# MMintLab/gelslim_depth

Hardware: AMD Instinct MI355X
Metric: train frames/sec (320x427) at batch 32 (higher is better)
Workload: dtype f32

## Files before the change

### gelslim_depth_amd/_lib.py

```python
from __future__ import annotations

import ctypes as C
import os
from typing import Optional, Sequence, Tuple

import torch

_HERE = os.path.dirname(os.path.abspath(__file__))
LIB_PATH = os.environ.get("GSD_LIB_PATH") or os.path.join(_HERE, "csrc", "libgsd.so")


class GsdError(RuntimeError):
    pass


class gsd_src(C.Structure):
    _fields_ = [("ptr", C.c_void_p), ("scale", C.c_void_p), ("shift", C.c_void_p),
                ("C", C.c_int32), ("H", C.c_int32), ("W", C.c_int32),
                ("off_h", C.c_int32), ("off_w", C.c_int32), ("relu", C.c_int32),
                ("w_stride", C.c_int32), ("slack", C.c_int32),
                ("n_stride", C.c_int64), ("c_stride", C.c_int64)]


class gsd_dst(C.Structure):
    _fields_ = [("ptr", C.c_void_p), ("C", C.c_int32), ("H", C.c_int32), ("W", C.c_int32),
                ("off_h", C.c_int32), ("off_w", C.c_int32), ("w_stride", C.c_int32),
                ("n_stride", C.c_int64), ("c_stride", C.c_int64)]


class gsd_guard(C.Structure):
    _fields_ = [("words", C.c_void_p), ("tick", C.c_int32)]


class gsd_nhwc(C.Structure):
    _fields_ = [("ptr", C.c_void_p), ("pitch", C.c_int64),
                ("N", C.c_int32), ("H", C.c_int32), ("W", C.c_int32), ("C", C.c_int32)]


_P = C.c_void_p
_I = C.c_int
_L = C.c_int64
_F = C.c_float
_D = C.c_double
_SRC = C.POINTER(gsd_src)
_DST = C.POINTER(gsd_dst)
_GUARD = C.POINTER(gsd_guard)
class gsd_bf16_bnbwd(C.Structure):
    _fields_ = [("y", C.POINTER(gsd_nhwc)), ("scale", C.c_void_p), ("shift", C.c_void_p), ("mean", C.c_void_p),
                ("invstd", C.c_void_p)]


class gsd_wl_job(C.Structure):
    _fields_ = [("w", C.c_void_p), ("wt", C.c_void_p), ("mode", C.c_int32), ("Co", C.c_int32), ("Ci", C.c_int32), ("reserved", C.c_int32)]


class gsd_bf16_wimg_job(C.Structure):
    _fields_ = [("w", C.c_void_p), ("out", C.c_void_p), ("mode", C.c_int32), ("Cout", C.c_int32), ("Cin", C.c_int32),
                ("reserved", C.c_int32)]


_NHWC = C.POINTER(gsd_nhwc)
_BNBWD = C.POINTER(gsd_bf16_bnbwd)
_IP = C.POINTER(C.c_int)

SIGNATURES = {
    "gsd_version": (C.c_char_p, []),
    "gsd_last_error": (C.c_char_p, []),
    "gsd_selftest_mfma": (_I, [_P, _P, _P, _P]),
    "gsd_weight_layout_size": (_L, [_I, _I, _I]),
    "gsd_weight_layout": (_I, [_I, _P, _I, _I, _P, _P]),
    "gsd_weight_layout_batch": (_I, [C.POINTER(gsd_wl_job), _I, _P]),
    "gsd_conv3x3_partial_rows": (_I, [_I, _I, _I, _I]),
    "gsd_conv3x3": (_I, [_SRC, _I, _P, _I, _I, _DST, _I, _P, _I, _I, _I, _P]),
    "gsd_conv3x3_dgrad_bnrelu": (_I, [_SRC, _P, _I, _I, _DST, _P, _P, _P, _P, _P, _P, _I, _I, _I, _P]),
    "gsd_conv3x3_algo": (_I, [_I, _I, _I, _I, _I]),
    "gsd_conv3x3_w43_partial_rows": (_I, [_I, _I, _I, _I]),
    "gsd_conv3x3_w43_mfma_count": (C.c_int64, [_I, _I, _I, _I, _I]),
    "gsd_conv3x3_w43": (_I, [_SRC, _I, _P, _I, _I, _DST, _I, _P, _I, _I, _I, _P]),
    "gsd_conv3x3_w43_dgrad_bnrelu": (_I, [_SRC, _P, _I, _I, _DST, _P, _P, _P, _P, _P, _P, _I, _I, _I, _P]),
    "gsd_conv3x3_w2d_supported": (_I, [_I, _I]),
    "gsd_conv3x3_prefers_w2d": (_I, [_I, _I, _I, _I, _I, _I]),
    "gsd_conv3x3_w2d_estimate_us": (C.c_double, [_I, _I, _I, _I, _I]),
    "gsd_conv3x3_w43_estimate_us": (C.c_double, [_I, _I, _I, _I, _I, _I]),
    "gsd_conv3x3_w2d_partial_rows": (_I, [_I, _I, _I, _I]),
    "gsd_conv3x3_w2d_mfma_count": (C.c_int64, [_I, _I, _I, _I, _I]),
    "gsd_conv3x3_w2d": (_I, [_SRC, _I, _P, _I, _I, _DST, _I, _P, _I, _I, _I, _P]),
    "gsd_conv3x3_w2d_dgrad_bnrelu": (_I, [_SRC, _P, _I, _I, _DST, _P, _P, _P, _P, _P, _P, _I, _I, _I, _P]),
    "gsd_conv3x3_w2d_estimate_slabs_us": (C.c_double, [_I, _I, _I, _I, _I]),
    "gsd_conv3x3_w2d_workspace": (_L, [_I, _I, _I, _I, _I]),
    "gsd_conv3x3_w2d_ws": (_I, [_SRC, _I, _P, _I, _I, _DST, _I, _P, _P, _L, _I, _I, _I, _P]),
    "gsd_conv3x3_w2d_dgrad_bnrelu_ws": (_I, [_SRC, _P, _I, _I, _DST, _P, _P, _P, _P, _P, _P, _P, _L, _I, _I, _I, _P]),
    "gsd_conv3x3_w43_workspace": (_L, [_I, _I, _I, _I, _I]),
    "gsd_conv3x3_w43_ws": (_I, [_SRC, _I, _P, _I, _I, _DST, _I, _P, _P, _L, _I, _I, _I, _P]),
    "gsd_conv3x3_w43_dgrad_bnrelu_ws": (_I, [_SRC, _P, _I, _I, _DST, _P, _P, _P, _P, _P, _P, _P, _L, _I, _I, _I, _P]),
    "gsd_convT2x2": (_I, [_SRC, _P, _P, _I, _I, _DST, _I, _I, _I, _P]),
    "gsd_convT2x2_dgrad_layout": (_I, [_SRC, _I, _I, _I, _I, _I]),
    "gsd_convT2x2_dgrad": (_I, [_SRC, _P, _I, _I, _DST, _I, _I, _I, _P]),
    "gsd_convT2x2_dgrad_as": (_I, [_I, _SRC, _P, _I, _I, _DST, _I, _I, _I, _P]),
    "gsd_convT2x2_dgrad_bnrelu_partial_rows": (_I, [_SRC, _I, _I, _I, _I, _I]),
    "gsd_convT2x2_dgrad_bnrelu": (_I, [_SRC, _P, _I, _I, _DST, _P, _P, _P, _P, _P, _P, _I, _I, _I, _P]),
    "gsd_conv3x3_wgrad_workspace": (_L, [_I, _I, _I, _I, _I]),
    "gsd_conv3x3_wgrad": (_I, [_SRC, _I, _SRC, _I, _I, _P, _P, _L, _I, _I, _I, _P]),
    "gsd_conv3x3_wgrad_form": (_I, [_SRC, _I, _SRC, _I, _I, _I, _I, _I]),
    "gsd_conv3x3_wgrad_mfma_count": (C.c_int64, [_I, _I, _I, _I, _I, _I]),
    "gsd_conv3x3_wgrad_takes_pitched_dy": (_I, [_I, _I, _I, _I, _I]),
    "gsd_conv3x3_wgrad_bn_supported": (_I, [_I, _I, _I, _I, _I]),
    "gsd_conv3x3_wgrad_bn_workspace": (_L, [_I, _I, _I, _I, _I]),
    "gsd_conv3x3_wgrad_bn": (_I, [_SRC, _P, _P, _P, _P, _P, _P, _P, _I, _I, _P, _P, _L, _I, _I, _I, _P]),
    "gsd_conv3x3_dgrad_bn_supported": (_I, [_I, _I, _I, _I, _I]),
    "gsd_conv3x3_dgrad_bn": (_I, [_P, _P, _P, _P, _P, _P, _P, _P, _I, _I, _P, _I, _I, _I, _P]),
    "gsd_convT2x2_wgrad_workspace": (_L, [_I, _I, _I, _I, _I]),
    "gsd_convT2x2_wgrad": (_I, [_SRC, _SRC, _I, _I, _P, _P, _P, _L, _I, _I, _I, _P]),
    "gsd_bn_reduce_partials": (_I, [_P, _I, _I, _I, _P, _P]),
    "gsd_partials_channel_sums": (_I, [_P, _I, _I, _I, _I, _I, _P, _P, _P]),
    "gsd_add_counters": (_I, [C.POINTER(C.c_void_p), _I, _L, _P]),
    "gsd_bn_finalize": (_I, [_P, _I, _D, _P, _P, _F, _F, _P, _P, _P, _P, _P, _P, _GUARD, _P]),
    "gsd_bn_eval_coeffs": (_I, [_P, _P, _P, _P, _F, _I, _P, _P, _P]),
    "gsd_bn_eval_coeffs_bwd": (_I, [_P, _P, _P, _P, _F, _I, _P, _P, _P, _P, _P]),
    "gsd_bn_bwd_partial_rows": (_I, [_I, _I, _I, _I]),
    "gsd_bn_bwd_reduce": (_I, [_I, _P, _P, _P, _P, _P, _SRC, _P, _P, _P, _I, _P, _P, _I, _I, _I, _I, _P]),
    "gsd_bn_bwd_reduce_partials": (_I, [_P, _I, _I, _P, _P]),
    "gsd_bn_bwd_finalize": (_I, [_P, _P, _I, _D, _P, _P, _P, _P, _P, _P]),
    "gsd_bn_bwd_apply": (_I, [_P, _P, _P, _P, _P, _P, _P, _I, _I, _I, _I, _P, _I, _P]),
    "gsd_sum_planes": (_I, [_P, _I, _I, _L, _P, _P, _P]),
    "gsd_maxpool2": (_I, [_SRC, _P, _I, _I, _I, _I, _P]),
    "gsd_conv1x1_out": (_I, [_SRC, _P, _P, _I, _I, _P, _I, _I, _I, _P]),
    "gsd_conv1x1_out_wgrad_rows": (_I, [_I, _I, _I]),
    "gsd_conv1x1_out_wgrad": (_I, [_P, _P, _P, _P, _I, _I, _P, _P, _P, _I, _I, _I, _P]),
    "gsd_loss_fwd_bwd": (_I, [_I, _P, _P, _L, _F, _P, _P, _P, _GUARD, _P]),
    "gsd_guard_snapshot": (_I, [_P, _P, _L, _P]),
    "gsd_guard_restore": (_I, [_GUARD, _P, _P, _L, _P]),
    "gsd_adam_ema": (_I, [_P, _P, _P, _P, _P, _L, _I, _F, _F, _F, _F, _F, _F, _F, _GUARD, _P]),
    "gsd_bn_reduce_finalize": (_I, [_P, _I, _I, _I, _P, _D, _P, _P, _F, _F, _P, _P, _P, _P, _P, _P, _GUARD, _P]),
    "gsd_bn_bwd_reduce_finalize": (_I, [_P, _I, _I, _I, _P, _D, _P, _P, _P, _P, _P, _P]),
    "gsd_area_resize_affine": (_I, [_P, _P, _I, _I, _I, _I, _P, _I, _I, _P, _P, _I, _F, _F, _P]),
    "gsd_ingest_images": (_I, [_P, _P, _I, _I, _I, _I, _I, _L, _L, _L, _L, _P, _I, _I, _F, _F, _P]),
    "gsd_resize_affine": (_I, [_I, _P, _P, _I, _I, _I, _I, _P, _I, _I, _P, _P, _I, _F, _F, _P]),
    "gsd_ingest_images_interp": (_I, [_I, _P, _P, _I, _I, _I, _I, _I, _L, _L, _L, _L, _P, _I, _I, _F, _F, _P]),
    "gsd_gaussian_blur": (_I, [_P, _L, _I, _I, _P, _I, _P, _P]),
    "gsd_channel_stats_workspace": (_L, [_I]),
    "gsd_channel_stats": (_I, [_P, _L, _I, _L, _P, _P, _P]),
    "gsd_gather_affine": (_I, [_P, _P, _L, _I, _I, _L, _P, _P, _I, _P, _P]),
    "gsd_bf16_conv_mpad": (_I, [_I]),
    "gsd_bf16_conv_partial_rows": (_I, [_I, _I, _I, _I]),
    "gsd_bf16_conv_dense_partial_rows": (_I, [_I, _I, _I, _I, _I, _I, _I]),
    "gsd_bf16_conv3x3": (_I, [_NHWC, _P, _NHWC, _I, _I, _P, _BNBWD, _P]),
    "gsd_bf16_conv_dense": (_I, [_NHWC, _P, _NHWC, _I, _I, _I, _I, _IP, _IP, _I, _I, _I, _I, _I, _P, _P, _BNBWD, _P]),
    "gsd_bf16_conv3x3_bnrelu": (_I, [_NHWC, _P, _NHWC, _I, _I, _P, _P, _P]),
    "gsd_bf16_conv1x1_bnrelu": (_I, [_NHWC, _P, _NHWC, _I, _I, _P, _P, _P]),
    "gsd_bf16_weight_image_size": (_L, [_I, _I, _I]),
    "gsd_bf16_weight_image": (_I, [_I, _P, _I, _I, _P, _P]),
    "gsd_bf16_weight_images": (_I, [C.POINTER(gsd_bf16_wimg_job), _I, _P]),
    "gsd_bf16_im2col3x3": (_I, [_P, _I, _I, _I, _I, _NHWC, _P]),
    "gsd_bf16_conv3x3_first_supported": (_I, [_I, _I]),
    "gsd_bf16_conv3x3_first_partial_rows": (_I, [_I, _I, _I, _I]),
    "gsd_bf16_conv3x3_first": (_I, [_P, _I, _I, _I, _I, _P, _NHWC, _I, _P, _P, _P, _P]),
    "gsd_bf16_wgrad_first_workspace": (_L, [_I, _I, _I, _I]),
    "gsd_bf16_wgrad_first": (_I, [_P, _I, _I, _I, _I, _NHWC, _NHWC, _P, _P, _P, _P, _P, _P, _P, _L, _P]),
    "gsd_bf16_inc_supported": (_I, [_I, _I]),
    "gsd_bf16_inc_conv_partial_rows": (_I, [_I, _I, _I]),
    "gsd_bf16_inc_conv": (_I, [_P, _I, _I, _I, _I, _P, _P, _P, _P, _NHWC, _NHWC, _P, _P]),
    "gsd_bf16_first_bn_bwd_reduce": (_I, [_P, _I, _I, _I, _I, _P, _NHWC, _P, _P, _P, _P, _P, _P]),
    "gsd_bf16_wgrad_first_recompute": (_I, [_P, _I, _I, _I, _I, _P, _NHWC, _P, _P, _P, _P, _P, _P, _P, _P, _L, _P]),
    "gsd_bf16_conv3x3_c64_supported": (_I, [_I, _I]),
    "gsd_bf16_conv3x3_c64_partial_rows": (_I, [_I, _I, _I]),
    "gsd_bf16_conv3x3_c64": (_I, [_NHWC, _P, _NHWC, _P, _BNBWD, _P]),
    "gsd_bf16_bn_apply": (_I, [_NHWC, _P, _P, _NHWC, _I, _P]),
    "gsd_bf16_bn_apply_pool": (_I, [_NHWC, _P, _P, _NHWC, _NHWC, _P]),
    "gsd_bf16_bn_apply_pool_idx": (_I, [_NHWC, _P, _P, _NHWC, _NHWC, _P, _P]),
    "gsd_bf16_bn_bwd_reduce_pool_idx": (_I, [_NHWC, _P, _P, _P, _P, _NHWC, _P, _NHWC, _NHWC, _P, _P]),
    "gsd_bf16_maxpool2": (_I, [_NHWC, _NHWC, _P]),
    "gsd_bf16_conv1x1_out": (_I, [_NHWC, _P, _P, _I, _P, _P]),
    "gsd_bf16_bn_relu_conv1x1_out": (_I, [_NHWC, _P, _P, _P, _P, _I, _P, _P]),
    "gsd_bf16_bn_bwd_partial_rows": (_I, [_I, _I, _I]),
    "gsd_bf16_bn_bwd_reduce": (_I, [_I, _NHWC, _P, _P, _P, _P, _NHWC, _NHWC, _NHWC, _P, _P, _NHWC, _P, _P]),
    "gsd_bf16_bn_bwd_apply": (_I, [_NHWC, _NHWC, _P, _P, _P, _P, _P, _P]),
    "gsd_bf16_channel_sums_workspace": (_L, [_I, _I, _I, _I]),
    "gsd_bf16_channel_sums": (_I, [_NHWC, _I, _I, _I, _I, _P, _P, _L, _P]),
    "gsd_bf16_convT_bias_grad_workspace": (_L, [_I, _I, _I, _I, _I, _I, _I, _I]),
    "gsd_bf16_convT_bias_grad": (_I, [_P, _I, _I, _I, _NHWC, _I, _I, _I, _I, _P, _P, _L, _P]),
    "gsd_bf16_wgrad_workspace": (_L, [_I, _I, _I, _I, _I, _I]),
    "gsd_bf16_wgrad": (_I, [_NHWC, _NHWC, _I, _I, _IP, _IP, _P, _I, _P, _L, _P]),
}


def _load() -> C.CDLL:
    if not os.path.exists(LIB_PATH):
        raise GsdError(
            f"{LIB_PATH} not found: build it first (python -c 'import __graft_entry__ as g; g.build()' "
            f"or python -m gelslim_depth_amd.build). There is no CPU/torch fallback for the hot path.")
    lib = C.CDLL(LIB_PATH)
    for name, (res, args) in SIGNATURES.items():
        fn = getattr(lib, name)
        fn.restype = res
        fn.argtypes = args
    return lib


lib = _load()


def check(rc: int, what: str = "") -> None:
    if rc != 0:
        msg = lib.gsd_last_error().decode("utf-8", "replace")
        raise GsdError(f"libgsd {what} failed (code {rc}): {msg}")


def version() -> str:
    return lib.gsd_version().decode()


def stream_ptr() -> int:
    return torch.cuda.current_stream().cuda_stream


def ptr(t: Optional[torch.Tensor]) -> Optional[int]:
    return None if t is None else t.data_ptr()


def _chk_f32(t: torch.Tensor) -> None:
    if t.dtype != torch.float32 or not t.is_cuda:
        raise GsdError(f"expected a float32 CUDA(HIP) tensor, got {t.dtype} on {t.device}")


def _nchw_strides(t: torch.Tensor) -> Tuple[int, int, int]:
    if t.dim() != 4:
        raise GsdError(f"expected an NCHW tensor, got shape {tuple(t.shape)}")
    n, c, h, w = t.shape
    if w > 1 and t.stride(3) != 1:
        raise GsdError(f"expected an NCHW tensor with unit column stride, got shape {tuple(t.shape)} strides {t.stride()}")
    ws = t.stride(2) if (h > 1 or t.stride(2) >= w) else w
    cs = t.stride(1) if (c > 1 or t.stride(1) >= h * ws) else h * ws
    ns = t.stride(0) if (n > 1 or t.stride(0) >= c * cs) else c * cs
    if ws < w or cs < h * ws or ns < c * cs:
        raise GsdError(f"expected an NCHW tensor with unit column stride, got shape {tuple(t.shape)} strides {t.stride()}")
    return ns, cs, ws


def _chk_nchw(t: torch.Tensor) -> None:
    _nchw_strides(t)


def pitched_empty(shape, device, pitch_multiple: int = 4) -> torch.Tensor:
    n, c, h, w = shape
    p = -(-w // pitch_multiple) * pitch_multiple
    return torch.empty((n, c, h, p), device=device, dtype=torch.float32)[..., :w]


def make_src(t: torch.Tensor, scale: Optional[torch.Tensor] = None, shift: Optional[torch.Tensor] = None,
             relu: bool = False, c_off: int = 0, c_len: Optional[int] = None,
             off: Tuple[int, int] = (0, 0), slack: int = 0) -> gsd_src:
    _chk_f32(t)
    ns, cs, ws = _nchw_strides(t)
    n, ct, h, w = t.shape
    cl = ct - c_off if c_len is None else c_len
    s = gsd_src()
    s.ptr = t.data_ptr() + 4 * c_off * cs
    s.scale = ptr(scale)
    s.shift = ptr(shift)
    s.C, s.H, s.W = cl, h, w
    s.off_h, s.off_w = off
    s.relu = 1 if relu else 0
    s.w_stride = ws
    s.slack = slack
    s.n_stride = ns
    s.c_stride = cs
    return s


SLACK = 4


def slack_empty(shape, device) -> torch.Tensor:
    numel = 1
    for d in shape:
        numel *= int(d)
    buf = torch.empty((numel + 2 * SLACK,), device=device, dtype=torch.float32)
    buf[:SLACK].zero_()
    buf[-SLACK:].zero_()
    return buf[SLACK:SLACK + numel].view(*shape)


def make_dst(t: torch.Tensor, c_off: int = 0, c_len: Optional[int] = None, off: Tuple[int, int] = (0, 0)) -> gsd_dst:
    _chk_f32(t)
    ns, cs, ws = _nchw_strides(t)
    n, ct, h, w = t.shape
    cl = ct - c_off if c_len is None else c_len
    d = gsd_dst()
    d.ptr = t.data_ptr() + 4 * c_off * cs
    d.C, d.H, d.W = cl, h, w
    d.off_h, d.off_w = off
    d.w_stride = ws
    d.n_stride = ns
    d.c_stride = cs
    return d


def make_nhwc(t: torch.Tensor, c_off: int = 0, c_len: Optional[int] = None) -> gsd_nhwc:
    if t.dtype != torch.bfloat16 or not t.is_cuda or t.dim() != 4 or not t.is_contiguous():
        raise GsdError(f"expected a contiguous (N,H,W,C) bfloat16 CUDA(HIP) tensor, got {t.dtype} {tuple(t.shape)} on {t.device}")
    n, h, w, ct = t.shape
    d = gsd_nhwc()
    d.ptr = t.data_ptr() + 2 * c_off
    d.pitch = ct
    d.N, d.H, d.W = n, h, w
    d.C = ct - c_off if c_len is None else c_len
    return d


def make_guard(words: Optional[torch.Tensor], tick: int):
    if words is None:
        return None
    if words.dtype != torch.int32 or not words.is_cuda or words.numel() < 2 or tick == 0:
        raise GsdError("a guard needs two int32 words on the GPU and a non-zero tick")
    g = gsd_guard()
    g.words = words.data_ptr()
    g.tick = tick
    return C.pointer(g)


def add_counters(tensors: Sequence[torch.Tensor], delta: int = 1) -> None:
    if not tensors:
        return
    for t in tensors:
        if t.dtype != torch.int64 or not t.is_cuda or t.numel() != 1:
            raise GsdError(f"add_counters: expected int64 scalars on the GPU, got {t.dtype} {tuple(t.shape)} on {t.device}")
    arr = (C.c_void_p * len(tensors))(*[t.data_ptr() for t in tensors])
    check(lib.gsd_add_counters(arr, len(tensors), delta, stream_ptr()), "add_counters")


def int_array(vals: Sequence[int]):
    return (C.c_int * len(vals))(*vals)


def src_array(items: Sequence[gsd_src]):
    arr = (gsd_src * len(items))()
    for i, it in enumerate(items):
        arr[i] = it
    return arr


def dst_array(items: Sequence[gsd_dst]):
    arr = (gsd_dst * len(items))()
    for i, it in enumerate(items):
        arr[i] = it
    return arr
```

### gelslim_depth_amd/csrc/gsd_conv3x3_w2d.hip

```cpp
#include "gsd_common.h"

#include <cstdio>
#include <cstdlib>
#include <type_traits>

__device__ const float gsd_pad_w2d[2] = {0.f, __builtin_nanf("")};

typedef float f32x4v __attribute__((ext_vector_type(4), aligned(4)));
typedef float f32x2v __attribute__((ext_vector_type(2)));

struct W2DParams {
  SrcD src0, src1;
  DstD dst0, dst1;
  const float* wt;
  float* partials;
  const float* bw_raw;
  const float* bw_scale;
  const float* bw_shift;
  const float* bw_mean;
  const float* bw_invstd;
  int Cin, Cout, Mpad, nchunks, mblocks;
  int N, H, W;
  int TH, TW, TWq, tiles_y, tiles_x, WR, WC, WCp, PS, NPV;
  int NP, NI;
  int mgrp, pgrp, ptiles;
  int nslab;
  float* slabs;
};

namespace {
constexpr int W2D_BM = 64;
constexpr int W2D_WTILE = 96 * W2D_BM;
constexpr int NWP = 2;
}

template <class GetY>
__device__ __forceinline__ void w2d_epilogue(const W2DParams& P, const float* sBw, const int n, const int h0, const int w0, const int tr2,
                                             const int tq, const int vmask, const int m0, const int mh, const int ph, const int j,
                                             const int l16, const int pt, GetY get_y) {
  constexpr int BM = 64;
  int off0_0 = 0, off0_1 = 0, off1_0 = 0, off1_1 = 0, sm0_0 = 0, sm0_1 = 0, sm1_0 = 0, sm1_1 = 0;
#pragma unroll
  for (int a = 0; a < 2; ++a) {
    const int h = h0 + 2 * tr2 + a, w = w0 + 4 * tq;
    const int vm = (vmask >> (4 * a)) & 15;
    int hd = h - P.dst0.oh, wd = w - P.dst0.ow;
    if ((unsigned)hd < (unsigned)P.dst0.H) {
      (a == 0 ? off0_0 : off0_1) = hd * P.dst0.ws + wd;
#pragma unroll
      for (int i = 0; i < 4; ++i)
        if ((vm >> i & 1) && (unsigned)(wd + i) < (unsigned)P.dst0.W) (a == 0 ? sm0_0 : sm0_1) |= 1 << i;
    }
    hd = h - P.dst1.oh;
    wd = w - P.dst1.ow;
    if ((unsigned)hd < (unsigned)P.dst1.H) {
      (a == 0 ? off1_0 : off1_1) = hd * P.dst1.ws + wd;
#pragma unroll
      for (int i = 0; i < 4; ++i)
        if ((vm >> i & 1) && (unsigned)(wd + i) < (unsigned)P.dst1.W) (a == 0 ? sm1_0 : sm1_1) |= 1 << i;
    }
  }
  auto OFF0 = [&](int a) { return a == 0 ? off0_0 : off0_1; };
  auto OFF1 = [&](int a) { return a == 0 ? off1_0 : off1_1; };
  auto SM0 = [&](int a) { return a == 0 ? sm0_0 : sm0_1; };
  auto SM1 = [&](int a) { return a == 0 ? sm1_0 : sm1_1; };
  const long long lane0 = (long long)(j * 4) * P.dst0.cs, lane1 = (long long)(j * 4) * P.dst1.cs;
  float* const d0 = P.dst0.p + (long long)n * P.dst0.ns;
  float* const d1 = P.dst1.p + (long long)n * P.dst1.ns;
  float* const prow = P.partials != nullptr ? P.partials + (size_t)(pt * NWP + ph) * (2 * P.Mpad) : nullptr;

  if (P.bw_raw == nullptr) {
#pragma unroll
    for (int m = 0; m < 2; ++m) {
#pragma unroll
      for (int reg = 0; reg < 4; ++reg) {
        const int cu = m0 + mh * 32 + m * 16 + reg, co = cu + j * 4;
        const bool first = co < P.dst0.C;
        const int cd = first ? co : co - P.dst0.C;
        const bool co_ok = co < P.Cout && (first || cd < P.dst1.C);
        float* const plane = first ? d0 + (long long)cu * P.dst0.cs + lane0 : d1 + (long long)(cu - P.dst0.C) * P.dst1.cs + lane1;
        float y[2][4];
        get_y(m, reg, y);
        float s1 = 0.f, s2 = 0.f;
#pragma unroll
        for (int a = 0; a < 2; ++a) {
          const int sm = co_ok ? (first ? SM0(a) : SM1(a)) : 0;
          float* const px = plane + (first ? OFF0(a) : OFF1(a));
#pragma unroll
          for (int i = 0; i < 4; ++i) {
            if (sm >> i & 1) {
              s1 += y[a][i];
              s2 = fmaf(y[a][i], y[a][i], s2);
            }
          }
          if (sm == 15) {
            *reinterpret_cast<f32x4v*>(px) = f32x4{y[a][0], y[a][1], y[a][2], y[a][3]};
          } else {
#pragma unroll
            for (int i = 0; i < 4; ++i)
              if (sm >> i & 1) px[i] = y[a][i];
          }
        }
        if (prow != nullptr) {
          s1 = reduce16_to_lane15(s1);
          s2 = reduce16_to_lane15(s2);
          if (l16 == 15 && co < P.Mpad) {
            prow[co] = s1;
            prow[P.Mpad + co] = s2;
          }
        }
      }
    }
  } else {
#pragma unroll
    for (int m = 0; m < 2; ++m) {
#pragma unroll
      for (int reg = 0; reg < 4; ++reg) {
        const int cu = m0 + mh * 32 + m * 16 + reg, co = cu + j * 4;
        const long long cplane = (long long)n * P.dst0.ns + (co < P.Cout ? (long long)cu * P.dst0.cs + lane0 : 0);
        float xr[2][4];
#pragma unroll
        for (int a = 0; a < 2; ++a) {
          const float* const rp = P.bw_raw + cplane + OFF0(a);
          if (SM0(a) == 15) {
            const f32x4 t = *reinterpret_cast<const f32x4v*>(rp);
            xr[a][0] = t[0], xr[a][1] = t[1], xr[a][2] = t[2], xr[a][3] = t[3];
          } else {
#pragma unroll
            for (int i = 0; i < 4; ++i) xr[a][i] = (SM0(a) >> i & 1) ? rp[i] : 0.f;
          }
        }
        const int cl = mh * 32 + m * 16 + j * 4 + reg;
        const float bsc = sBw[cl], bsh = sBw[BM + cl], bmu = sBw[2 * BM + cl], bis = sBw[3 * BM + cl];
        float y[2][4];
        get_y(m, reg, y);
        float s1 = 0.f, s2 = 0.f;
#pragma unroll
        for (int a = 0; a < 2; ++a) {
          const int sm = co < P.Cout ? SM0(a) : 0;
          float* const px = d0 + ((long long)cu * P.dst0.cs + lane0) + OFF0(a);
#pragma unroll
          for (int i = 0; i < 4; ++i) {
            const float x = xr[a][i];
            const float dz = ((sm >> i & 1) && fmaf(x, bsc, bsh) > 0.f) ? y[a][i] : 0.f;
            y[a][i] = dz;
            s1 += dz;
            s2 = fmaf(dz, (x - bmu) * bis, s2);
          }
          if (sm == 15) {
            *reinterpret_cast<f32x4v*>(px) = f32x4{y[a][0], y[a][1], y[a][2], y[a][3]};
          } else {
#pragma unroll
            for (int i = 0; i < 4; ++i)
              if (sm >> i & 1) px[i] = y[a][i];
          }
        }
        if (prow != nullptr) {
          s1 = reduce16_to_lane15(s1);
          s2 = reduce16_to_lane15(s2);
          if (l16 == 15 && co < P.Mpad) {
            prow[co] = s1;
            prow[P.Mpad + co] = s2;
          }
        }
      }
    }
  }
}

template <bool PLAIN, int HM = 0, bool SPLIT = false>
__global__ __launch_bounds__(128 * NWP, 2) void conv3x3_w2d_kernel(const W2DParams P) {
  constexpr bool X4 = HM == 1, U4 = HM == 2, PC = HM != 0;
  constexpr int W2D_NONE = -2147483647 - 1, W2D_PAD = -2147483647;
  static_assert(!X4 || PLAIN, "aligned 16-byte halo pieces: a plain, row-pitched source");
  constexpr int BM = W2D_BM, WTILE = W2D_WTILE, NT = 128 * NWP, NW = 2 * NWP;
  extern __shared__ __attribute__((aligned(16))) float smem[];
  const int PS = P.PS;
  const int BUF = WTILE + 4 * PS;

  const int tid = threadIdx.x, lane = tid & 63;
  const int wave8 = __builtin_amdgcn_readfirstlane(tid >> 6);
  const int ph = wave8 % NWP, fh = wave8 / NWP;
  const int j = lane >> 4, l16 = lane & 15;

  const int lid = xcd_swizzle(blockIdx.x, gridDim.x);
  int mbb = lid % P.mblocks;
  const int slab = SPLIT ? (lid / P.mblocks) % P.nslab : 0;
  int pt = SPLIT ? lid / P.mblocks / P.nslab : lid / P.mblocks;
  if (!SPLIT && P.mgrp < P.mblocks) {
    const int gsz = P.pgrp * P.mblocks;
    const int g = lid / gsz;
    int r = lid - g * gsz;
    const int p0 = g * P.pgrp;
    const int pn = min(P.pgrp, P.ptiles - p0);
    const int per = pn * P.mgrp;
    const int mg = r / per;
    r -= mg * per;
    const int gn = min(P.mgrp, P.mblocks - mg * P.mgrp);
    const int pl = r / gn;
    pt = p0 + pl;
    mbb = mg * P.mgrp + (r - pl * gn);
  }
  const int c_lo = SPLIT ? (int)((long)slab * P.nchunks / P.nslab) : 0;
  const int c_hi = SPLIT ? (int)((long)(slab + 1) * P.nchunks / P.nslab) : P.nchunks;
  const int m0 = mbb * BM;
  const int tpi = P.tiles_y * P.tiles_x;
  const int n = pt / tpi;
  const int rt = pt - n * tpi;
  const int ty = rt / P.tiles_x;
  const int h0 = ty * P.TH, w0 = (rt - ty * P.tiles_x) * P.TW;

  const int q = ph * 16 + l16;
  const bool q_ok = q < (P.TH >> 1) * P.TWq && q < 16 * NWP;
  const int tr2 = q_ok ? q / P.TWq : 0;
  const int tq = q_ok ? q - tr2 * P.TWq : 0;
  const int baddr = WTILE + j * PS + (2 * tr2) * P.WCp + 4 * tq + (PC ? 4 : 0);
  int vmask = 0;
  if (q_ok) {
#pragma unroll
    for (int a = 0; a < 2; ++a)
      if (h0 + 2 * tr2 + a < P.H) {
#pragma unroll
        for (int i = 0; i < 4; ++i)
          if (w0 + 4 * tq + i < P.W) vmask |= 1 << (4 * a + i);
      }
  }

  bool p_on[2];
  int pmask = 0;
  auto seg_offsets = [&](const int seg, int (&xo)[2], const bool mark) __attribute__((always_inline)) {
    const SrcD& S = seg ? P.src1 : P.src0;
#pragma unroll
    for (int pp = 0; pp < 2; ++pp) {
      xo[pp] = W2D_NONE;
      if constexpr (PC) {
        const int u = wave8 + NW * pp;
        p_on[pp] = u < 4 * P.NI;
        const int piece = (u % P.NI) * 64 + lane;
        const int rr = piece / P.NP, pc = piece - rr * P.NP;
        if (rr < P.WR) {
          const int gh = h0 - 1 + rr, gw = w0 - 4 + 4 * pc;
          if constexpr (X4) {
            xo[pp] = ((unsigned)gh < (unsigned)S.H && gw >= 0 && gw + 4 <= S.ws) ? gh * S.ws + gw : W2D_PAD;
          } else {
            const int hs = gh - S.oh, c0 = gw - S.ow;
            xo[pp] = W2D_PAD;
            if (S.C > 0 && (unsigned)hs < (unsigned)S.H && c0 + 3 >= 0 && c0 < S.W) {
              xo[pp] = hs * S.ws + c0;
#pragma unroll
              for (int e = 0; e < 4; ++e)
                if (mark && (c0 + e < 0 || c0 + e >= S.W)) pmask |= 1 << (8 * seg + 4 * pp + e);
            }
          }
        }
        continue;
      }
      p_on[pp] = wave8 + NW * pp < P.NPV;
      const int pos = (wave8 + NW * pp) * 64 + lane;
      const int rr = pos / P.WCp, cc = pos - rr * P.WCp;
      if (rr < P.WR && cc < P.WC) {
        const int gh = h0 - 1 + rr, gw = w0 - 1 + cc;
        const int hs = gh - S.oh, ws = gw - S.ow;
        xo[pp] = ((unsigned)hs < (unsigned)S.H && (unsigned)ws < (unsigned)S.W) ? hs * S.ws + ws : W2D_PAD;
      }
    }
  };
  int xo0[2], xo1[2];
  seg_offsets(0, xo0, true);
  seg_offsets(1, xo1, true);
  const int f_sw = P.src1.C > 0 ? P.src0.C / 4 : -1;
  const bool start1 = SPLIT && f_sw >= 0 && c_lo >= f_sw;
  {
    const float pad0 = (start1 ? P.src1.relu : P.src0.relu) ? __builtin_nanf("") : 0.f;
#pragma unroll
    for (int pp = 0; pp < 2; ++pp)
      if (p_on[pp] && (start1 ? xo1[pp] : xo0[pp]) == W2D_PAD) {
#pragma unroll
        for (int b = 0; b < 2; ++b) {
          if constexpr (PC) {
            const int u = wave8 + NW * pp;
#pragma unroll
            for (int e = 0; e < 4; ++e) smem[b * BUF + WTILE + (u / P.NI) * PS + 1 + (u % P.NI) * 256 + lane * 4 + e] = pad0;
          } else {
#pragma unroll
            for (int ch = 0; ch < 4; ++ch) smem[b * BUF + WTILE + ch * PS + (wave8 + NW * pp) * 64 + lane] = pad0;
          }
        }
      }
  }
  long long d_cs = start1 ? P.src1.cs : P.src0.cs;
  const float* d_base = (start1 ? P.src1.p + (long long)n * P.src1.ns : P.src0.p + (long long)n * P.src0.ns) +
                        (long long)(c_lo - (start1 ? f_sw : 0)) * 4 * d_cs;
  long long f_xl[2];
#pragma unroll
  for (int pp = 0; pp < 2; ++pp) f_xl[pp] = start1 ? xo1[pp] : xo0[pp];
  auto begin_fill = [&](int chunk, int buf) {
    if (f_sw < 0 || start1 || (chunk != f_sw && chunk != f_sw + 1)) return;
    if (chunk == f_sw) {
      d_base = P.src1.p + (long long)n * P.src1.ns;
      d_cs = P.src1.cs;
      int xs[2];
      seg_offsets(1, xs, false);
#pragma unroll
      for (int pp = 0; pp < 2; ++pp) f_xl[pp] = xs[pp];
    }
    const float pad1 = P.src1.relu ? __builtin_nanf("") : 0.f;
#pragma unroll
    for (int pp = 0; pp < 2; ++pp)
      if (p_on[pp] && f_xl[pp] == W2D_PAD) {
        if constexpr (PC) {
          const int u = wave8 + NW * pp;
#pragma unroll
          for (int e = 0; e < 4; ++e) smem[buf * BUF + WTILE + (u / P.NI) * PS + 1 + (u % P.NI) * 256 + lane * 4 + e] = pad1;
        } else {
#pragma unroll
          for (int ch = 0; ch < 4; ++ch) smem[buf * BUF + WTILE + ch * PS + (wave8 + NW * pp) * 64 + lane] = pad1;
        }
      }
  };
  auto halo_slot = [&](int ch, float* Xb) {
#pragma unroll
    for (int pp = 0; pp < 2; ++pp)
      if (p_on[pp] && f_xl[pp] > W2D_PAD) __builtin_amdgcn_global_load_lds(d_base + f_xl[pp], Xb + ch * PS + (wave8 + NW * pp) * 64, 4, 0, 0);
    d_base += d_cs;
  };
  auto halo_unit = [&](int pp, float* Xb) {
    const int u = wave8 + NW * pp;
    if (p_on[pp] && f_xl[pp] > W2D_PAD)
      __builtin_amdgcn_global_load_lds(d_base + (u / P.NI) * d_cs + f_xl[pp], Xb + (u / P.NI) * PS + 1 + (u % P.NI) * 256, 16, 0, 0);
    if (pp == 1) d_base += 4 * d_cs;
  };
  constexpr int WPW = 24 / NW;
  const float* const wsrc0 = P.wt + (size_t)mbb * P.nchunks * WTILE + wave8 * (WPW * 256) + lane * 4;
  auto weight_fill = [&](int chunk, float* Wn) {
    const float* wg = wsrc0 + (size_t)chunk * WTILE;
    float* wl = Wn + wave8 * (WPW * 256);
    __builtin_amdgcn_global_load_lds(wg, wl, 16, 0, 0);
    __builtin_amdgcn_global_load_lds(wg, wl, 16, 1024, 0);
    __builtin_amdgcn_global_load_lds(wg, wl, 16, 2048, 0);
    if constexpr (WPW == 6) {
      __builtin_amdgcn_global_load_lds(wg, wl, 16, 3072, 0);
      __builtin_amdgcn_global_load_lds(wg + 1024, wl + 1024, 16, 0, 0);
      __builtin_amdgcn_global_load_lds(wg + 1024, wl + 1024, 16, 1024, 0);
    }
  };

  const int Kpad = P.nchunks * 4;
  float* sAff = smem + 2 * BUF;
  for (int c = tid; c < Kpad; c += NT) {
    const bool first = c < P.src0.C;
    const SrcD& S = first ? P.src0 : P.src1;
    const int cc = first ? c : c - P.src0.C;
    float sc = 1.f, sh = 0.f;
    if (c < P.Cin && cc < S.C && S.scale != nullptr) {
      sc = S.scale[cc];
      sh = S.shift[cc];
    }
    sAff[c] = sc;
    sAff[Kpad + c] = sh;
  }
  float* sBw = sAff + 2 * Kpad;
  if (P.bw_raw != nullptr) {
    for (int c = tid; c < BM; c += NT) {
      const int co = m0 + c < P.Cout ? m0 + c : 0;
      sBw[c] = P.bw_scale[co];
      sBw[BM + c] = P.bw_shift[co];
      sBw[2 * BM + c] = P.bw_mean[co];
      sBw[3 * BM + c] = P.bw_invstd[co];
    }
  }
  const float lo0 = P.src0.relu ? 0.f : -__builtin_inff(), lo1 = P.src1.relu ? 0.f : -__builtin_inff();

  const int rowA = baddr + (fh ? 2 : 0) * P.WCp, rowB = baddr + (fh ? 1 : 2) * P.WCp, rowC = baddr + (fh ? 3 : 1) * P.WCp;
  const f32x2v sg2 = {fh ? -1.f : 1.f, fh ? -1.f : 1.f};

  f32x4 acc[4][12];
#pragma unroll
  for (int m = 0; m < 4; ++m)
#pragma unroll
    for (int f = 0; f < 12; ++f) acc[m][f] = f32x4{0.f, 0.f, 0.f, 0.f};

  const int a_keep = (j * 12 + fh * 6) * 128 + l16 * 4 + fh * 64, a_give = a_keep + (fh ? -64 : 64);
  begin_fill(c_lo, 0);
  weight_fill(c_lo, smem);
  if constexpr (PC) {
    halo_unit(0, smem + WTILE);
    halo_unit(1, smem + WTILE);
  } else {
#pragma unroll
    for (int ch = 0; ch < 4; ++ch) halo_slot(ch, smem + WTILE);
  }

  auto run_chunk = [&](const int chunk, auto cur_c) {
    constexpr int cur = decltype(cur_c)::value;
    if constexpr (U4) {
      __builtin_amdgcn_s_waitcnt(0x0F70);
      const bool seg1 = f_sw >= 0 && chunk >= f_sw;
      const int pm = seg1 ? pmask >> 8 : pmask & 0xff;
      if (pm != 0) {
        const float padv = (seg1 ? P.src1.relu : P.src0.relu) ? __builtin_nanf("") : 0.f;
#pragma unroll
        for (int pp = 0; pp < 2; ++pp) {
          const int u = wave8 + NW * pp;
          float* pq = smem + cur * BUF + WTILE + (u / P.NI) * PS + 1 + (u % P.NI) * 256 + lane * 4;
#pragma unroll
          for (int e = 0; e < 4; ++e)
            if (pm >> (4 * pp + e) & 1) pq[e] = padv;
        }
      }
      __syncthreads();
    } else {
      gsd_dma_barrier();
    }
    const int kc = chunk * 4 + j;
    float sc = 1.f, sh = 0.f, lo = 0.f;
    if constexpr (!PLAIN) {
      sc = sAff[kc], sh = sAff[Kpad + kc];
      lo = kc < P.src0.C ? lo0 : (kc < P.Cin ? lo1 : -__builtin_inff());
    }
    const bool more = chunk + 1 < c_hi;
    int ioff = cur * BUF;
    __asm__ volatile("" : "+s"(ioff));
    const float* Wc = smem + ioff;
    auto load_row = [&](const int addr, float (&r)[6]) {
      const f32x4 ra = *reinterpret_cast<const f32x4*>(&Wc[addr]);
      const f32x2v rb = *reinterpret_cast<const f32x2v*>(&Wc[addr + 4]);
      r[0] = ra[0], r[1] = ra[1], r[2] = ra[2], r[3] = ra[3], r[4] = rb[0], r[5] = rb[1];
    };
    float dA[6], dB[6], dC[6];
    load_row(rowA, dA);
    load_row(rowB, dB);
    load_row(rowC, dC);
    f32x4 av[2];
    av[0] = *reinterpret_cast<const f32x4*>(&Wc[a_keep]);
    auto affine = [&](float (&r)[6]) {
      if constexpr (!PLAIN) {
        const f32x2v sc2 = {sc, sc}, sh2 = {sh, sh};
#pragma unroll
        for (int c = 0; c < 6; c += 2) {
          const f32x2v y = __builtin_elementwise_fma(f32x2v{r[c], r[c + 1]}, sc2, sh2);
          r[c] = fmaxf(y[0], lo);
          r[c + 1] = fmaxf(y[1], lo);
        }
      }
    };
    const f32x2v m41 = {-4.f, -1.f}, p1m1 = {1.f, -1.f}, p2m2 = {2.f, -2.f}, m5 = {-5.f, -5.f}, p4 = {4.f, 4.f};
    auto rt_a = [&](const f32x2v (&tp)[3], f32x2v& ac, f32x2v& be) {
      ac = __builtin_elementwise_fma(f32x2v{tp[1][0], tp[1][0]}, m41, f32x2v{tp[2][0], tp[2][0]});
      be = __builtin_elementwise_fma(f32x2v{tp[0][1], tp[0][1]}, m41, f32x2v{tp[1][1], tp[1][1]});
    };
    auto rt_b = [&](const f32x2v& ac, const f32x2v& be, float (&v)[6]) {
      const f32x2v v12 = __builtin_elementwise_fma(f32x2v{be[0], be[0]}, p1m1, f32x2v{ac[0], ac[0]});
      const f32x2v v34 = __builtin_elementwise_fma(f32x2v{be[1], be[1]}, p2m2, f32x2v{ac[1], ac[1]});
      v[1] = v12[0], v[2] = v12[1], v[3] = v34[0], v[4] = v34[1];
    };
    auto rt_c = [&](const f32x2v (&tp)[3], float (&v)[6]) {
      const f32x2v v05 = __builtin_elementwise_fma(tp[0], p4, __builtin_elementwise_fma(tp[1], m5, tp[2]));
      v[0] = v05[0], v[5] = v05[1];
    };
    affine(dA);
    affine(dB);
    f32x2v tA[3], tB[3], acB, beB;
#pragma unroll
    for (int k = 0; k < 3; ++k) tA[k] = f32x2v{dA[2 * k], dA[2 * k + 1]} - f32x2v{dB[2 * k], dB[2 * k + 1]};
    auto col_b = [&]() {
#pragma unroll
      for (int k = 0; k < 3; ++k)
        tB[k] = __builtin_elementwise_fma(f32x2v{dC[2 * k], dC[2 * k + 1]}, sg2, f32x2v{dB[2 * k], dB[2 * k + 1]});
    };
    if constexpr (!PLAIN) {
      affine(dC);
      col_b();
    }
    float v[2][6];
    {
      f32x2v ac, be;
      rt_a(tA, ac, be);
      rt_b(ac, be, v[0]);
      rt_c(tA, v[0]);
    }
    __builtin_amdgcn_sched_barrier(0);
#pragma unroll
    for (int g = 0; g < 12; ++g) {
      const int r = g / 6, fe = (g >> 1) * 2 - 6 * r, mt = 2 * (g & 1);
      if (g + 1 < 12) av[(g + 1) & 1] = *reinterpret_cast<const f32x4*>(&Wc[((g + 1) & 1 ? a_give : a_keep) + ((g + 1) >> 1) * 128]);
      const f32x4& ap = av[g & 1];
      acc[mt][6 * r + fe] = mfma16(ap[0], v[r][fe], acc[mt][6 * r + fe]);
      acc[mt + 1][6 * r + fe] = mfma16(ap[1], v[r][fe], acc[mt + 1][6 * r + fe]);
      acc[mt][6 * r + fe + 1] = mfma16(ap[2], v[r][fe + 1], acc[mt][6 * r + fe + 1]);
      acc[mt + 1][6 * r + fe + 1] = mfma16(ap[3], v[r][fe + 1], acc[mt + 1][6 * r + fe + 1]);
      const int piece = PLAIN ? g + 1 : g + 2;
      if (piece == 1) col_b();
      if (piece == 2) rt_a(tB, acB, beB);
      if (piece == 3) rt_b(acB, beB, v[1]);
      if (piece == 4) rt_c(tB, v[1]);
      if (more && g < 3) {
        float* Wn = smem + (cur ^ 1) * BUF;
        if (g == 0) {
          begin_fill(chunk + 1, cur ^ 1);
          weight_fill(chunk + 1, Wn);
        } else {
          if constexpr (PC) {
            halo_unit(g - 1, Wn + WTILE);
          } else {
            halo_slot(2 * g - 2, Wn + WTILE);
            halo_slot(2 * g - 1, Wn + WTILE);
          }
        }
      }
      if (g < 6) {
#pragma unroll
        for (int i = 0; i < 4; ++i) {
          __builtin_amdgcn_sched_group_barrier(0x008, 1, 0);
          __builtin_amdgcn_sched_group_barrier(0x002, 1, 0);
        }
      }
      __builtin_amdgcn_sched_barrier(0);
    }
  };
  for (int chunk = c_lo; chunk < c_hi; chunk += 2) {
    run_chunk(chunk, std::integral_constant<int, 0>{});
    if (chunk + 1 < c_hi) run_chunk(chunk + 1, std::integral_constant<int, 1>{});
  }

  {
    float* const xs = smem + (wave8 * 12) * 256 + lane * 4;
    const float* const xr = smem + ((ph + NWP * (1 - fh)) * 12) * 256 + lane * 4;
#pragma unroll
    for (int r = 0; r < 2; ++r) {
      __syncthreads();
#pragma unroll
      for (int f = 0; f < 12; ++f) *reinterpret_cast<f32x4*>(xs + f * 256) = acc[2 + r][f];
      __syncthreads();
#pragma unroll
      for (int f = 0; f < 12; ++f) acc[2 + r][f] = *reinterpret_cast<const f32x4*>(xr + f * 256);
    }
  }

  auto out_transform = [&](auto hi_c, int m, int reg, float (&y)[2][4]) __attribute__((always_inline)) {
    constexpr bool HI = decltype(hi_c)::value;
    const int lo = HI ? 2 + m : m, hi = HI ? m : 2 + m;
    const int r0 = reg & ~1;
#pragma unroll
    for (int a = 0; a < 2; ++a) {
      f32x2v R[6];
#pragma unroll
      for (int fc = 0; fc < 6; ++fc) {
        const f32x2v M0 = {acc[lo][fc][r0], acc[lo][fc][r0 + 1]}, M1 = {acc[lo][6 + fc][r0], acc[lo][6 + fc][r0 + 1]};
        const f32x2v M2 = {acc[hi][fc][r0], acc[hi][fc][r0 + 1]}, M3 = {acc[hi][6 + fc][r0], acc[hi][6 + fc][r0 + 1]};
        R[fc] = a == 0 ? M0 + M1 + M2 : M1 - M2 - M3;
      }
      const f32x2v p12 = R[1] + R[2], m12 = R[1] - R[2], p34 = R[3] + R[4], m34 = R[3] - R[4];
      const f32x2v c2 = {2.f, 2.f}, c4 = {4.f, 4.f}, c8 = {8.f, 8.f};
      const f32x2v y0 = R[0] + p12 + p34, y1 = __builtin_elementwise_fma(c2, m34, m12), y2 = __builtin_elementwise_fma(c4, p34, p12);
      const f32x2v y3 = __builtin_elementwise_fma(c8, m34, m12) + R[5];
      y[a][0] = y0[reg & 1], y[a][1] = y1[reg & 1], y[a][2] = y2[reg & 1], y[a][3] = y3[reg & 1];
    }
  };

  auto finish = [&](auto hi_c) __attribute__((always_inline)) {
    auto get_y = [&](int m, int reg, float (&y)[2][4]) __attribute__((always_inline)) { out_transform(hi_c, m, reg, y); };
    if constexpr (SPLIT) {
      float* const sl = P.slabs + ((size_t)((size_t)pt * P.nslab + slab) * P.mblocks + mbb) * (size_t)(BM * 128 * NWP);
#pragma unroll
      for (int m = 0; m < 2; ++m)
#pragma unroll
        for (int reg = 0; reg < 4; ++reg) {
          float y[2][4];
          get_y(m, reg, y);
          float* const o = sl + ((size_t)(fh * 32 + m * 16 + j * 4 + reg) * (16 * NWP) + q) * 8;
          *reinterpret_cast<f32x4*>(o) = f32x4{y[0][0], y[0][1], y[0][2], y[0][3]};
          *reinterpret_cast<f32x4*>(o + 4) = f32x4{y[1][0], y[1][1], y[1][2], y[1][3]};
        }
    } else {
      w2d_epilogue(P, sBw, n, h0, w0, tr2, tq, vmask, m0, fh, ph, j, l16, pt, get_y);
    }
  };
  if (fh == 0)
    finish(std::false_type{});
  else
    finish(std::true_type{});
}

__global__ __launch_bounds__(128 * NWP) void w2d_slab_reduce_kernel(const W2DParams P) {
  constexpr int BM = W2D_BM;
  __shared__ float sBw[4 * BM];
  const int tid = threadIdx.x, lane = tid & 63;
  const int wave8 = __builtin_amdgcn_readfirstlane(tid >> 6);
  const int ph = wave8 % NWP, mh = wave8 / NWP;
  const int j = lane >> 4, l16 = lane & 15;
  const int lid = xcd_swizzle(blockIdx.x, gridDim.x);
  const int mbb = lid % P.mblocks;
  const int pt = lid / P.mblocks;
  const int m0 = mbb * BM;
  const int tpi = P.tiles_y * P.tiles_x;
  const int n = pt / tpi;
  const int rt = pt - n * tpi;
  const int ty = rt / P.tiles_x;
  const int h0 = ty * P.TH, w0 = (rt - ty * P.tiles_x) * P.TW;
  const int q = ph * 16 + l16;
  const bool q_ok = q < (P.TH >> 1) * P.TWq && q < 16 * NWP;
  const int tr2 = q_ok ? q / P.TWq : 0;
  const int tq = q_ok ? q - tr2 * P.TWq : 0;
  int vmask = 0;
  if (q_ok) {
#pragma unroll
    for (int a = 0; a < 2; ++a)
      if (h0 + 2 * tr2 + a < P.H) {
#pragma unroll
        for (int i = 0; i < 4; ++i)
          if (w0 + 4 * tq + i < P.W) vmask |= 1 << (4 * a + i);
      }
  }
  if (P.bw_raw != nullptr) {
    for (int c = tid; c < BM; c += 128 * NWP) {
      const int co = m0 + c < P.Cout ? m0 + c : 0;
      sBw[c] = P.bw_scale[co];
      sBw[BM + c] = P.bw_shift[co];
      sBw[2 * BM + c] = P.bw_mean[co];
      sBw[3 * BM + c] = P.bw_invstd[co];
    }
    __syncthreads();
  }
  const size_t tile_elems = (size_t)(BM * 128 * NWP);
  const float* const s0 = P.slabs + ((size_t)pt * P.nslab * P.mblocks + mbb) * tile_elems;
  auto get_y = [&](int m, int reg, float (&y)[2][4]) __attribute__((always_inline)) {
    const float* o = s0 + ((size_t)(mh * 32 + m * 16 + j * 4 + reg) * (16 * NWP) + q) * 8;
    f32x4 a = *reinterpret_cast<const f32x4*>(o), b = *reinterpret_cast<const f32x4*>(o + 4);
    for (int s = 1; s < P.nslab; ++s) {
      o += (size_t)P.mblocks * tile_elems;
      a += *reinterpret_cast<const f32x4*>(o);
      b += *reinterpret_cast<const f32x4*>(o + 4);
    }
    y[0][0] = a[0], y[0][1] = a[1], y[0][2] = a[2], y[0][3] = a[3];
    y[1][0] = b[0], y[1][1] = b[1], y[1][2] = b[2], y[1][3] = b[3];
  };
  w2d_epilogue(P, sBw, n, h0, w0, tr2, tq, vmask, m0, mh, ph, j, l16, pt, get_y);
}

namespace {

struct W2DPlan {
  int TH, TW, TWq, tiles_y, tiles_x, mblocks, WR, WC, WCp, PS;
};

int w2d_read_cycles(int TWq, int LP, int PS) {
  static const int g128[2][16] = {{0, 1, 2, 3, 12, 13, 14, 15, 20, 21, 22, 23, 24, 25, 26, 27},
                                  {4, 5, 6, 7, 8, 9, 10, 11, 16, 17, 18, 19, 28, 29, 30, 31}};
  int total = 0;
  for (int ph = 0; ph < NWP; ++ph) {
    int addr[64];
    for (int lane = 0; lane < 64; ++lane) {
      const int q = ph * 16 + (lane & 15);
      addr[lane] = (lane >> 4) * PS + 2 * (q / TWq) * LP + 4 * (q % TWq);
    }
    for (int half = 0; half < 2; ++half) {
      for (int g = 0; g < 2; ++g) {
        int worst = 0;
        for (int slot = 0; slot < 16; ++slot) {
          int distinct = 0, seen[16];
          for (int i = 0; i < 16; ++i) {
            const int a = addr[g128[g][i] + 32 * half];
            if ((a / 4) % 16 != slot) continue;
            bool dup = false;
            for (int k = 0; k < distinct; ++k) dup = dup || seen[k] == a;
            if (!dup) seen[distinct++] = a;
          }
          worst = distinct > worst ? distinct : worst;
        }
        total += worst;
      }
      int worst = 0;
      for (int slot = 0; slot < 32; ++slot) {
        int distinct = 0, seen[32];
        for (int i = 0; i < 32; ++i) {
          const int a = addr[i + 32 * half] + 4;
          if ((a / 2) % 32 != slot) continue;
          bool dup = false;
          for (int k = 0; k < distinct; ++k) dup = dup || seen[k] == a;
          if (!dup) seen[distinct++] = a;
        }
        worst = distinct > worst ? distinct : worst;
      }
      total += worst;
    }
  }
  return total;
}

bool plan_w2d(int N, int H, int W, int M, W2DPlan* best) {
  long best_cost = -1;
  const int force_tw = gsd_env_int("GSD_W2D_TW", 0);
  const int maxpos = 256 * NWP;
  static const int tws[4] = {32, 64, 16, 8};
  for (int k = 0; k < 4; ++k) {
    const int tw = tws[k];
    if (force_tw && tw != force_tw) continue;
    const int twq = tw / 4;
    int th = 2 * (16 * NWP / twq);
    const int wcp0 = round_up(tw + 2, 4);
    if ((th + 2) * wcp0 > maxpos) continue;
    const int ty = ceil_div(H, th);
    th = round_up(ceil_div(H, ty), 2);
    const long blocks = (long)ty * ceil_div(W, tw) * N;
    const long cost = (blocks * 8 + (tw == 32 ? 0 : tw == 64 ? 1 : tw == 16 ? 2 : 3)) * (tw == 8 ? 100 + gsd_env_int("GSD_W2D_TW8_PCT", 8) : 100);
    if (best_cost < 0 || cost < best_cost) {
      best_cost = cost;
      best->TH = th; best->TW = tw; best->TWq = twq;
      best->tiles_y = ty; best->tiles_x = ceil_div(W, tw);
      best->WR = th + 2; best->WC = tw + 2;
    }
  }
  best->mblocks = ceil_div(M, W2D_BM);
  if (best_cost < 0) return false;
  static std::atomic<uint64_t> memo[16];
  const int th = best->TH, tw = best->TW, key = (th << 16) | (tw << 4);
  std::atomic<uint64_t>& mm = memo[(th * 7 + tw) & 15];
  {
    const uint64_t v = mm.load(std::memory_order_acquire);
    if (v != 0 && (int)(v >> 40) == key) {
      best->WCp = (int)(v >> 20) & 0xFFFFF;
      best->PS = (int)v & 0xFFFFF;
      return true;
    }
  }
  const int wcp0 = round_up(tw + 2, 4);
  int bc = -1;
  for (int c = wcp0; c <= wcp0 + 12 && (th + 2) * c <= maxpos; c += 4)
    for (int ps = round_up((th + 2) * c, 4) + 4; ps < round_up((th + 2) * c, 4) + 4 + 36; ps += 4) {
      const int cyc = w2d_read_cycles(best->TWq, c, ps);
      if (bc < 0 || cyc < bc) {
        bc = cyc;
        best->WCp = c;
        best->PS = ps;
      }
    }
  if (key < (1 << 24) && best->WCp < (1 << 20) && best->PS < (1 << 20))
    mm.store(((uint64_t)key << 40) | ((uint64_t)best->WCp << 20) | (uint64_t)best->PS, std::memory_order_release);
  return true;
}

int w2d_x4_plane_stride(int TWq, int WCp, int WR) {
  static std::atomic<uint64_t> memo[8];
  const int key = (TWq << 20) | (WCp << 8) | WR;
  std::atomic<uint64_t>& mm = memo[(TWq + WR) & 7];
  {
    const uint64_t v = mm.load(std::memory_order_acquire);
    if (v != 0 && (int)(v >> 32) == key) return (int)(v & 0xFFFFFFFFu);
  }
  int best = -1, ps_best = WR * WCp + 4;
  for (int ps = WR * WCp + 4; ps < WR * WCp + 4 + 68; ps += 4) {
    const int c = w2d_read_cycles(TWq, WCp, ps);
    if (best < 0 || c < best) {
      best = c;
      ps_best = ps;
    }
  }
  mm.store(((uint64_t)(unsigned)key << 32) | (uint64_t)(unsigned)ps_best, std::memory_order_release);
  return ps_best;
}

template <bool PLAIN, int HM = 0, bool SPLIT = false>
int launch_w2d(const W2DParams& P, int grid, size_t lds, hipStream_t st) {
  static gsd_attr_once big_lds;
  const void* fn = reinterpret_cast<const void*>(&conv3x3_w2d_kernel<PLAIN, HM, SPLIT>);
  if (hipError_t e = gsd_allow_big_lds(big_lds, fn); e != hipSuccess) {
    gsd_set_error("gsd_conv3x3_w2d: hipFuncSetAttribute: %s", hipGetErrorString(e));
    return GSD_ERR_HIP;
  }
  GSD_REQUIRE(lds <= 160 * 1024, GSD_ERR_UNSUPPORTED, "gsd_conv3x3_w2d: LDS image %zu B too large", lds);
  hipLaunchKernelGGL((conv3x3_w2d_kernel<PLAIN, HM, SPLIT>), dim3(grid), dim3(128 * NWP), lds, st, P);
  GSD_LAUNCH_CHECK("gsd_conv3x3_w2d");
  if constexpr (SPLIT) {
    hipLaunchKernelGGL(w2d_slab_reduce_kernel, dim3(grid / P.nslab), dim3(128 * NWP), 0, st, P);
    GSD_LAUNCH_CHECK("gsd_conv3x3_w2d (slab sums)");
  }
  return GSD_OK;
}

double w2d_time_us(long base, int nchunks, int S, bool bw) {
  const long cus = gsd_cu_count();
  const long k = (base * S + cus - 1) / cus;
  const double cu = (double)(k / 2) + (k & 1 ? 0.66 : 0.0);
  double t = cu * (2.07 * nchunks / S + 5.0);
  if (S > 1) t += 12.0 + (double)(S + 1 + (bw ? 1 : 0)) * base * 65536.0 / 6.0e6;
  return t;
}

int w2d_pick_slabs(long base, int nchunks, bool bw) {
  const int forced = gsd_env_int("GSD_W2D_SPLIT", -1);
  if (forced == 0 || forced == 1) return 1;
  int best = 1;
  double tb = w2d_time_us(base, nchunks, 1, bw) * (forced > 1 ? 1e9 : 0.97);
  for (int S = 2; S <= 8 && nchunks / S >= 8; ++S) {
    if (forced > 1 && S != forced) continue;
    const double t = w2d_time_us(base, nchunks, S, bw);
    if (t < tb) {
      tb = t;
      best = S;
    }
  }
  return best;
}

}

extern "C" int gsd_conv3x3_w2d_supported(int Cin, int C0) {
  return (Cin > 0 && Cin % 4 == 0 && C0 > 0 && C0 <= Cin && C0 % 4 == 0) ? 1 : 0;
}

extern "C" int gsd_conv3x3_w2d_partial_rows(int N, int H, int W, int Cout) {
  if (N <= 0 || H <= 0 || W <= 0 || Cout <= 0) return 0;
  W2DPlan p;
  if (!plan_w2d(N, H, W, Cout, &p)) return 0;
  return N * p.tiles_y * p.tiles_x * NWP;
}

extern "C" int64_t gsd_conv3x3_w2d_mfma_count(int N, int H, int W, int Cin, int Cout) {
  W2DPlan p;
  if (N <= 0 || H <= 0 || W <= 0 || Cin <= 0 || Cout <= 0 || !plan_w2d(N, H, W, Cout, &p)) return 0;
  return (int64_t)N * p.tiles_y * p.tiles_x * p.mblocks * ceil_div(Cin, 4) * (2 * NWP * 48);
}

extern "C" double gsd_conv3x3_w2d_estimate_us(int N, int H, int W, int Cin, int Cout) {
  W2DPlan p;
  if (N <= 0 || H <= 0 || W <= 0 || Cin <= 0 || Cout <= 0 || !plan_w2d(N, H, W, Cout, &p)) return 0.0;
  const long blocks = (long)N * p.tiles_y * p.tiles_x * p.mblocks;
  return w2d_time_us(blocks, ceil_div(Cin, 4), 1, false);
}

extern "C" double gsd_conv3x3_w2d_estimate_slabs_us(int N, int H, int W, int Cin, int Cout) {
  W2DPlan p;
  if (N <= 0 || H <= 0 || W <= 0 || Cin <= 0 || Cout <= 0 || !plan_w2d(N, H, W, Cout, &p)) return 0.0;
  const long blocks = (long)N * p.tiles_y * p.tiles_x * p.mblocks;
  return w2d_time_us(blocks, ceil_div(Cin, 4), w2d_pick_slabs(blocks, ceil_div(Cin, 4), false), false);
}

extern "C" int64_t gsd_conv3x3_w2d_workspace(int N, int H, int W, int Cin, int Cout) {
  W2DPlan p;
  if (N <= 0 || H <= 0 || W <= 0 || Cin <= 0 || Cout <= 0 || Cin % 4 != 0 || !plan_w2d(N, H, W, Cout, &p)) return 0;
  const long blocks = (long)N * p.tiles_y * p.tiles_x * p.mblocks;
  const int S = std::max(w2d_pick_slabs(blocks, Cin / 4, false), w2d_pick_slabs(blocks, Cin / 4, true));
  return S > 1 ? (int64_t)blocks * S * (W2D_BM * 256) : 0;
}

extern "C" double gsd_conv3x3_w43_estimate_us(int N, int H, int W, int Cin, int Cout, int slabs);

extern "C" int gsd_conv3x3_prefers_w2d(int N, int H, int W, int Cin, int Cout, int train) {
  if (N <= 0 || H <= 0 || W <= 0 || Cin < 16 || Cin % 4 != 0 || Cout <= 0) return 0;
  const int forced = gsd_env_int("GSD_CONV_W2D", -1);
  if (forced == 0 || forced == 1) return forced;
  if (!train) return 1;
  const double a = gsd_conv3x3_w2d_estimate_slabs_us(N, H, W, Cin, Cout), b = gsd_conv3x3_w43_estimate_us(N, H, W, Cin, Cout, 1);
  return a > 0.0 && b > 0.0 && a < b ? 1 : 0;
}

static int w2d_impl(const gsd_src* src, int nsrc, const float* wt, int Cin, int Cout, const gsd_dst* dst, int ndst, float* partials,
                    const float* bw_raw, const float* bw_scale, const float* bw_shift, const float* bw_mean, const float* bw_invstd,
                    int N, int H, int W, void* stream, float* ws = nullptr, int64_t ws_elems = 0) {
  GSD_REQUIRE(src && dst && wt, GSD_ERR_BAD_ARG, "gsd_conv3x3_w2d: null argument");
  GSD_REQUIRE(nsrc >= 1 && nsrc <= 2 && ndst >= 1 && ndst <= 2, GSD_ERR_BAD_ARG, "gsd_conv3x3_w2d: nsrc/ndst must be 1 or 2");
  GSD_REQUIRE(N > 0 && H > 0 && W > 0 && Cin > 0 && Cout > 0, GSD_ERR_BAD_ARG, "gsd_conv3x3_w2d: bad sizes");
  GSD_REQUIRE(H < 32768 && W < 32768, GSD_ERR_UNSUPPORTED, "gsd_conv3x3_w2d: H, W must be < 32768");
  GSD_REQUIRE(((uintptr_t)wt & 15) == 0, GSD_ERR_BAD_ARG, "gsd_conv3x3_w2d: weight layout must be 16-byte aligned");
  GSD_REQUIRE(gsd_conv3x3_w2d_supported(Cin, src[0].C), GSD_ERR_UNSUPPORTED,
              "gsd_conv3x3_w2d: Cin=%d and the first segment's %d channels must be multiples of 4 (use gsd_conv3x3_w43)", Cin, src[0].C);
  int csum = 0;
  for (int i = 0; i < nsrc; ++i) {
    if (int e = gsd_check_src(src[i], "gsd_conv3x3_w2d src", true)) return e;
    GSD_REQUIRE(src[i].scale == nullptr || src[i].relu != 0, GSD_ERR_UNSUPPORTED,
                "gsd_conv3x3_w2d: an affine source segment must also have relu (zero padding uses a NaN sentinel)");
    GSD_REQUIRE((int64_t)src[i].H * src[i].w_stride < (1LL << 31), GSD_ERR_UNSUPPORTED, "gsd_conv3x3_w2d: plane too large");
    csum += src[i].C;
  }
  GSD_REQUIRE(csum == Cin, GSD_ERR_BAD_ARG, "gsd_conv3x3_w2d: source segments hold %d channels, Cin=%d", csum, Cin);
  csum = 0;
  for (int i = 0; i < ndst; ++i) {
    if (int e = gsd_check_dst(dst[i], "gsd_conv3x3_w2d dst", true)) return e;
    GSD_REQUIRE((int64_t)dst[i].H * dst[i].w_stride < (1LL << 31), GSD_ERR_UNSUPPORTED, "gsd_conv3x3_w2d: plane too large");
    csum += dst[i].C;
  }
  GSD_REQUIRE(csum == Cout, GSD_ERR_BAD_ARG, "gsd_conv3x3_w2d: destination segments hold %d channels, Cout=%d", csum, Cout);

  W2DPlan pl;
  GSD_REQUIRE(plan_w2d(N, H, W, Cout, &pl), GSD_ERR_UNSUPPORTED, "gsd_conv3x3_w2d: no tile shape");
  W2DParams P;
  P.src0 = to_srcd(src[0]);
  P.src1 = nsrc > 1 ? to_srcd(src[1]) : null_srcd();
  P.dst0 = to_dstd(dst[0]);
  P.dst1 = ndst > 1 ? to_dstd(dst[1]) : null_dstd();
  P.wt = wt;
  P.partials = partials;
  P.bw_raw = bw_raw; P.bw_scale = bw_scale; P.bw_shift = bw_shift; P.bw_mean = bw_mean; P.bw_invstd = bw_invstd;
  P.Cin = Cin; P.Cout = Cout;
  P.Mpad = round_up(Cout, 64);
  P.nchunks = Cin / 4;
  P.mblocks = pl.mblocks;
  P.N = N; P.H = H; P.W = W;
  P.TH = pl.TH; P.TW = pl.TW; P.TWq = pl.TWq; P.tiles_y = pl.tiles_y; P.tiles_x = pl.tiles_x;
  P.WR = pl.WR; P.WC = pl.WC; P.WCp = pl.WCp; P.PS = pl.PS;
  P.NPV = ceil_div(P.WR * P.WCp, 64);
  GSD_REQUIRE(P.NPV <= 4 * NWP, GSD_ERR_UNSUPPORTED, "gsd_conv3x3_w2d: halo window too large");
  {
    int g = (gsd_env_int("GSD_W2D_L2KB", 3072) << 10) / (P.nchunks * W2D_WTILE * 4);
    const int forced = gsd_env_int("GSD_W2D_MGROUP", -1);
    if (forced == 0) g = P.mblocks;
    if (forced > 0) g = forced;
    P.mgrp = std::min(std::max(g, 1), P.mblocks);
    P.pgrp = std::max(gsd_env_int("GSD_W2D_PGROUP", 64 / P.mgrp), 1);
    P.ptiles = N * pl.tiles_y * pl.tiles_x;
  }
  const long base = (long)N * pl.tiles_y * pl.tiles_x * P.mblocks;
  int S = ws != nullptr ? w2d_pick_slabs(base, P.nchunks, bw_raw != nullptr) : 1;
  while (S > 1 && (int64_t)base * S * (W2D_BM * 256) > ws_elems) --S;
  if (S > 1 && P.nchunks / S < 2) S = 1;
  P.nslab = S;
  P.slabs = S > 1 ? ws : nullptr;
  if (S > 1) GSD_REQUIRE(((uintptr_t)ws & 15) == 0, GSD_ERR_BAD_ARG, "gsd_conv3x3_w2d: the K-slab workspace must be 16-byte aligned");
  const long grid = base * S;
  GSD_REQUIRE(grid < 2147483647L, GSD_ERR_UNSUPPORTED, "gsd_conv3x3_w2d: grid too large");
  bool plain = true;
  for (int i = 0; i < nsrc; ++i) plain = plain && src[i].scale == nullptr && src[i].relu == 0;
  P.NP = pl.TW / 4 + 2;
  P.NI = ceil_div(P.WR * P.NP, 64);
  const bool x4 = plain && nsrc == 1 && 4 * P.NI <= 8 && gsd_env_int("GSD_W2D_X4", 1) != 0 &&
                  ((uintptr_t)src[0].ptr & 15) == 0 && src[0].w_stride % 4 == 0 && src[0].c_stride % 4 == 0 && src[0].n_stride % 4 == 0 &&
                  src[0].off_h == 0 && src[0].off_w == 0 && src[0].w_stride >= round_up(src[0].W, 4);
  bool u4 = !x4 && 4 * P.NI <= 8 && gsd_env_int("GSD_W2D_U4", 1) != 0;
  for (int i = 0; i < nsrc && u4; ++i) u4 = src[i].slack >= 4;
  if (x4 || u4) {
    P.WCp = 4 * P.NP;
    P.PS = w2d_x4_plane_stride(pl.TWq, P.WCp, P.WR);
  }
  const size_t lds = (size_t)(2 * (W2D_WTILE + 4 * P.PS) + 2 * 4 * P.nchunks + 4 * W2D_BM) * sizeof(float);
  if (gsd_env_set("GSD_W2D_TRACE"))
    fprintf(stderr, "w2d M%d K%d %dx%d N%d nsrc %d ndst %d plain %d x4 %d u4 %d | ptr&15 %d ws %d cs%%4 %d ns%%4 %d NI %d tile %dx%d slabs %d\n", Cout, Cin, H, W, N,
            nsrc, ndst, (int)plain, (int)x4, (int)u4, (int)((uintptr_t)src[0].ptr & 15), src[0].w_stride, (int)(src[0].c_stride % 4),
            (int)(src[0].n_stride % 4), P.NI, pl.TH, pl.TW, S);
  if (S > 1) {
    if (x4) return launch_w2d<true, 1, true>(P, (int)grid, lds, (hipStream_t)stream);
    if (u4) return plain ? launch_w2d<true, 2, true>(P, (int)grid, lds, (hipStream_t)stream) : launch_w2d<false, 2, true>(P, (int)grid, lds, (hipStream_t)stream);
    return plain ? launch_w2d<true, 0, true>(P, (int)grid, lds, (hipStream_t)stream) : launch_w2d<false, 0, true>(P, (int)grid, lds, (hipStream_t)stream);
  }
  if (x4) return launch_w2d<true, 1>(P, (int)grid, lds, (hipStream_t)stream);
  if (u4) return plain ? launch_w2d<true, 2>(P, (int)grid, lds, (hipStream_t)stream) : launch_w2d<false, 2>(P, (int)grid, lds, (hipStream_t)stream);
  return plain ? launch_w2d<true>(P, (int)grid, lds, (hipStream_t)stream) : launch_w2d<false>(P, (int)grid, lds, (hipStream_t)stream);
}

extern "C" int gsd_conv3x3_w2d(const gsd_src* src, int nsrc, const float* wt, int Cin, int Cout, const gsd_dst* dst, int ndst,
                               float* partials, int N, int H, int W, void* stream) {
  return w2d_impl(src, nsrc, wt, Cin, Cout, dst, ndst, partials, nullptr, nullptr, nullptr, nullptr, nullptr, N, H, W, stream);
}

extern "C" int gsd_conv3x3_w2d_dgrad_bnrelu(const gsd_src* src, const float* wt, int Cin, int Cout, const gsd_dst* dst,
                                            const float* raw, const float* scale, const float* shift, const float* mean,
                                            const float* invstd, float* partials, int N, int H, int W, void* stream) {
  GSD_REQUIRE(dst && raw && scale && shift && mean && invstd && partials, GSD_ERR_BAD_ARG,
              "gsd_conv3x3_w2d_dgrad_bnrelu: null argument");
  GSD_REQUIRE(dst->C == Cout && dst->H == H && dst->W == W && dst->off_h == 0 && dst->off_w == 0, GSD_ERR_BAD_ARG,
              "gsd_conv3x3_w2d_dgrad_bnrelu: dst must be the full (Cout,H,W) gradient buffer (raw shares its strides)");
  return w2d_impl(src, 1, wt, Cin, Cout, dst, 1, partials, raw, scale, shift, mean, invstd, N, H, W, stream);
}

extern "C" int gsd_conv3x3_w2d_ws(const gsd_src* src, int nsrc, const float* wt, int Cin, int Cout, const gsd_dst* dst, int ndst,
                                  float* partials, float* workspace, int64_t workspace_elems, int N, int H, int W, void* stream) {
  return w2d_impl(src, nsrc, wt, Cin, Cout, dst, ndst, partials, nullptr, nullptr, nullptr, nullptr, nullptr, N, H, W, stream, workspace,
                  workspace_elems);
}

extern "C" int gsd_conv3x3_w2d_dgrad_bnrelu_ws(const gsd_src* src, const float* wt, int Cin, int Cout, const gsd_dst* dst,
                                               const float* raw, const float* scale, const float* shift, const float* mean,
                                               const float* invstd, float* partials, float* workspace, int64_t workspace_elems, int N,
                                               int H, int W, void* stream) {
  GSD_REQUIRE(dst && raw && scale && shift && mean && invstd && partials, GSD_ERR_BAD_ARG,
              "gsd_conv3x3_w2d_dgrad_bnrelu: null argument");
  GSD_REQUIRE(dst->C == Cout && dst->H == H && dst->W == W && dst->off_h == 0 && dst->off_w == 0, GSD_ERR_BAD_ARG,
              "gsd_conv3x3_w2d_dgrad_bnrelu: dst must be the full (Cout,H,W) gradient buffer (raw shares its strides)");
  return w2d_impl(src, 1, wt, Cin, Cout, dst, 1, partials, raw, scale, shift, mean, invstd, N, H, W, stream, workspace, workspace_elems);
}
```

### gelslim_depth_amd/engine.py

```python
from __future__ import annotations

import ctypes as C
import os
from typing import Callable, Dict, List, Optional, Sequence, Tuple

import torch

from . import _lib as L
from ._lib import lib, check

BN_EPS = 1e-5
BN_MOMENTUM = 0.1
GSD_ERR_UNSUPPORTED = -2


def _r64(c: int) -> int:
    return (c + 63) // 64 * 64


def _r4(w: int) -> int:
    return (w + 3) // 4 * 4


class _ConvForm:

    def __init__(self, algo: int):
        self.algo = algo
        self.conv = (lib.gsd_conv3x3, lib.gsd_conv3x3_w43, lib.gsd_conv3x3_w2d)[algo]
        self.dgrad_bnrelu = (lib.gsd_conv3x3_dgrad_bnrelu, lib.gsd_conv3x3_w43_dgrad_bnrelu, lib.gsd_conv3x3_w2d_dgrad_bnrelu)[algo]
        self.partial_rows = (lib.gsd_conv3x3_partial_rows, lib.gsd_conv3x3_w43_partial_rows, lib.gsd_conv3x3_w2d_partial_rows)[algo]
        self.mode_f, self.mode_d = ((0, 1), (4, 5), (8, 9))[algo]
        self.workspace = (lambda *a: 0, lib.gsd_conv3x3_w43_workspace, lib.gsd_conv3x3_w2d_workspace)[algo]

    @staticmethod
    def choose(n: int, h: int, w: int, cin: int, c0: int, cout: int, train: bool) -> "_ConvForm":
        if not train:
            algo = lib.gsd_conv3x3_algo(1, h, w, cin, cout)
            if algo == 1:
                algo = 2 if lib.gsd_conv3x3_w2d_supported(cin, c0) else 0
            return _ConvForm(algo)
        algo = lib.gsd_conv3x3_algo(n, h, w, cin, cout)
        if algo == 1 and lib.gsd_conv3x3_w2d_supported(cin, c0) and lib.gsd_conv3x3_prefers_w2d(n, h, w, cin, cout, int(train)):
            algo = 2
        return _ConvForm(algo)

    def run(self, ws, src, nsrc, wt, cin, cout, dst, ndst, part, n, h, w, st):
        if self.algo >= 1 and ws is not None:
            fn = lib.gsd_conv3x3_w43_ws if self.algo == 1 else lib.gsd_conv3x3_w2d_ws
            return fn(src, nsrc, wt, cin, cout, dst, ndst, part, ws.data_ptr(), ws.numel(), n, h, w, st)
        return self.conv(src, nsrc, wt, cin, cout, dst, ndst, part, n, h, w, st)

    def run_bnrelu(self, ws, src, wt, cin, cout, dst, raw, scale, shift, mean, invstd, part, n, h, w, st):
        if self.algo >= 1 and ws is not None:
            fn = lib.gsd_conv3x3_w43_dgrad_bnrelu_ws if self.algo == 1 else lib.gsd_conv3x3_w2d_dgrad_bnrelu_ws
            return fn(src, wt, cin, cout, dst, raw, scale, shift, mean, invstd, part, ws.data_ptr(), ws.numel(), n, h, w, st)
        return self.dgrad_bnrelu(src, wt, cin, cout, dst, raw, scale, shift, mean, invstd, part, n, h, w, st)


class _Unit:

    def __init__(self, prefix: str, conv_idx: int, bn_idx: int, cin: int, cout: int, level: int):
        self.prefix, self.conv_idx, self.bn_idx = prefix, conv_idx, bn_idx
        self.cin, self.cout, self.level = cin, cout, level
        self.wname = f"{prefix}.double_conv.{conv_idx}.weight"
        bn = f"{prefix}.double_conv.{bn_idx}."
        self.gname, self.bname = bn + "weight", bn + "bias"
        self.rmname, self.rvname, self.nbtname = bn + "running_mean", bn + "running_var", bn + "num_batches_tracked"
        self.need_dgrad = True
        self.c0 = cin
        self.wt_f = self.wt_d = None
        self.scale = self.shift = self.mean = self.invstd = self.c1 = self.c2 = None
        self.sums = None
        self.raw = self.g = None
        self.dsrc = None
        self.pitched = False
        self.fused_dw = False
        self.srcs = None
        self.form_f = self.form_d = None
        self.forms_f = None
        self.fused_rows = 0


class _Up:

    def __init__(self, j: int, cin: int, level_in: int):
        self.j, self.cin, self.cout, self.level_in = j, cin, cin // 2, level_in
        self.wname, self.bname = f"up.{j}.up.weight", f"up.{j}.up.bias"
        self.wt_f = self.wt_d = None
        self.mode_d = 3
        self.bn_rows = 0
        self.out = self.dout = None


class UNetEngine:
    def __init__(self, n_channels: int, n_classes: int, layer_dimensions: Sequence[int]):
        dims = list(layer_dimensions)
        self.n_channels, self.n_classes, self.dims = n_channels, n_classes, dims
        self.L = len(dims) - 1
        self.enc: List[Tuple[_Unit, _Unit]] = []
        self.dec: List[Tuple[_Unit, _Unit]] = []
        self.ups: List[_Up] = []
        self.enc.append((_Unit("inc", 0, 1, n_channels, dims[0], 0), _Unit("inc", 3, 4, dims[0], dims[0], 0)))
        self.enc[0][0].need_dgrad = False
        for i in range(self.L):
            p = f"down.{i}.maxpool_conv.1"
            self.enc.append((_Unit(p, 0, 1, dims[i], dims[i + 1], i + 1), _Unit(p, 3, 4, dims[i + 1], dims[i + 1], i + 1)))
        for j, i in enumerate(range(self.L, 0, -1)):
            cin, cout = dims[i], dims[i - 1]
            if dims[i - 1] + cin // 2 != cin:
                raise ValueError(f"layer_dimensions {dims}: level {i} needs dims[i-1] + dims[i]//2 == dims[i] "
                                 "(the reference model fails at torch.cat/conv otherwise)")
            self.ups.append(_Up(j, cin, i))
            p = f"up.{j}.conv"
            self.dec.append((_Unit(p, 0, 1, cin, cout, i - 1), _Unit(p, 3, 4, cout, cout, i - 1)))
            self.dec[-1][0].c0 = dims[i - 1]
        self.units: List[_Unit] = [u for pair in self.enc for u in pair] + [u for pair in self.dec for u in pair]
        self._shape = None
        self._dev = None
        self.sync_fn: Optional[Callable[[torch.Tensor], None]] = None
        self.world = 1
        self._saved = False
        self._saved_eval = False
        self.block_done_cb: Optional[Callable[[str], None]] = None
        self._nbt: list = []
        self.guard = None
        self.generation = 0
        self.one_launch_rows = int(os.environ.get("GSD_BN_ONE_LAUNCH_ROWS", "4096"))
        self.side_dw = os.environ.get("GSD_SIDE_DW", "1") != "0"
        self.side: Optional[torch.cuda.Stream] = None
        self._handoff: Optional[torch.cuda.Stream] = None
        self.kernel_log: Optional[list] = None
        self.wgrad_log: Optional[list] = None
        self.region_log: Optional[list] = None

    _SIZING_ENV = ("GSD_W2D_TW", "GSD_W2D_TW8_PCT", "GSD_W43_TW", "GSD_W43_FOLD", "GSD_CONV_W2D", "GSD_CONV_ALGO", "GSD_W43_SPLIT",
                   "GSD_WGRAD_ALGO", "GSD_WGRAD_W2D", "GSD_WG2D_KX", "GSD_WG2D_BLOCKS", "GSD_WGRAD_BLOCKS", "GSD_WG43_TW")

    def _ensure(self, n: int, h: int, w: int, dev: torch.device, train: bool) -> None:
        key = (n, h, w, str(dev), tuple(os.environ.get(k) for k in self._SIZING_ENV))
        if self._shape == key and (not train or self.units[0].g is not None):
            return
        if self._shape != key:
            for u in self.units:
                u.raw = u.g = None
            for up in self.ups:
                up.out = up.dout = None
        self._shape = key
        self._dev = dev
        hs, ws = [h], [w]
        for _ in range(self.L):
            hs.append(hs[-1] // 2)
            ws.append(ws[-1] // 2)
        assert hs[-1] >= 1 and ws[-1] >= 1, "input too small for this many max-pools"
        self.hs, self.ws = hs, ws
        f32 = dict(device=dev, dtype=torch.float32)
        max_part = 1
        max_ws = 1
        max_gp = 0
        max_slab = 0
        for u in self.units:
            lh, lw = hs[u.level], ws[u.level]
            if u.raw is None:
                u.raw = L.slack_empty((n, u.cout, lh, lw), dev)
            if train and u.g is None:
                u.g = torch.empty((n, u.cout, lh, lw), **f32)
            if u.scale is None or u.scale.device != dev:
                for nm in ("scale", "shift", "mean", "invstd", "c1", "c2"):
                    setattr(u, nm, torch.empty((u.cout,), **f32))
                u.sums = torch.empty((65 * 3 * u.cout,), device=dev, dtype=torch.float64)
            u.forms_f = {t: _ConvForm.choose(n, lh, lw, u.cin, u.c0, u.cout, t) for t in (False, True)}
            u.form_f = u.forms_f[train]
            u.form_d = _ConvForm.choose(n, lh, lw, u.cout, u.cout, u.cin, True) if u.need_dgrad else None
            need = max(lib.gsd_weight_layout_size(f.mode_f, u.cout, u.cin) for f in u.forms_f.values())
            if u.wt_f is None or u.wt_f.numel() != need or u.wt_f.device != dev:
                u.wt_f = torch.empty((need,), **f32)
            if not u.need_dgrad and train:
                need = lib.gsd_weight_layout_size(1, u.cout, u.cin)
                if u.wt_d is None or u.wt_d.numel() != need or u.wt_d.device != dev:
                    u.wt_d = torch.empty((need,), **f32)
            if u.need_dgrad:
                need = lib.gsd_weight_layout_size(u.form_d.mode_d, u.cout, u.cin)
                if u.wt_d is None or u.wt_d.numel() != need or u.wt_d.device != dev:
                    u.wt_d = torch.empty((need,), **f32)
                max_part = max(max_part, u.form_d.partial_rows(n, lh, lw, u.cin) * 2 * _r64(u.cin))
            rows = max(f.partial_rows(n, lh, lw, u.cout) for f in u.forms_f.values())
            max_part = max(max_part, rows * 2 * _r64(u.cout))
            if train:
                max_slab = max(max_slab, u.form_f.workspace(n, lh, lw, u.cin, u.cout),
                               u.form_d.workspace(n, lh, lw, u.cout, u.cin) if u.need_dgrad else 0)
                max_part = max(max_part, lib.gsd_bn_bwd_partial_rows(n, u.cout, lh, lw) * 3 * u.cout)
                max_ws = max(max_ws, lib.gsd_conv3x3_wgrad_workspace(n, lh, lw, u.cin, u.cout))
                u.pitched = bool(lib.gsd_conv3x3_wgrad_takes_pitched_dy(n, lh, lw, u.cin, u.cout)) and \
                    (not u.need_dgrad or u.form_d.algo >= 1)
                if u.pitched:
                    max_gp = max(max_gp, n * u.cout * lh * _r4(lw))
                u.fused_dw = (not u.need_dgrad) and bool(lib.gsd_conv3x3_wgrad_bn_supported(n, lh, lw, u.cin, u.cout))
                if u.fused_dw:
                    max_ws = max(max_ws, lib.gsd_conv3x3_wgrad_bn_workspace(n, lh, lw, u.cin, u.cout))
        for up in self.ups:
            li = up.level_in
            if up.out is None:
                up.out = L.slack_empty((n, up.cout, 2 * hs[li], 2 * ws[li]), dev)
            if train and up.dout is None:
                up.dout = L.slack_empty((n, up.cout, 2 * hs[li], 2 * ws[li]), dev)
            if up.wt_f is None or up.wt_f.device != dev:
                up.wt_f = torch.empty((lib.gsd_weight_layout_size(6, up.cout, up.cin),), **f32)
            if train:
                up.mode_d = lib.gsd_convT2x2_dgrad_layout(C.byref(L.make_src(up.dout, slack=L.SLACK)), up.cin, up.cout, n, hs[li], ws[li])
                need = lib.gsd_weight_layout_size(up.mode_d, up.cout, up.cin)
                if up.wt_d is None or up.wt_d.numel() != need or up.wt_d.device != dev:
                    up.wt_d = torch.empty((need,), **f32)
                up.bn_rows = 0
                if up.mode_d == 7:
                    up.bn_rows = lib.gsd_convT2x2_dgrad_bnrelu_partial_rows(C.byref(L.make_src(up.dout, slack=L.SLACK)), up.cin,
                                                                            up.cout, n, hs[li], ws[li])
                    max_part = max(max_part, up.bn_rows * 2 * _r64(up.cin))
            if train:
                max_ws = max(max_ws, lib.gsd_convT2x2_wgrad_workspace(n, hs[li], ws[li], up.cin, up.cout))
        self.pooled = [None] + [L.slack_empty((n, self.dims[l - 1], hs[l], ws[l]), dev) for l in range(1, self.L + 1)]
        self.dpooled = [None] + ([torch.empty((n, self.dims[l - 1], hs[l], ws[l]), **f32)
                                 for l in range(1, self.L + 1)] if train else [None] * self.L)
        side = train and self.side_dw
        self.side = torch.cuda.Stream(device=dev) if side else None
        self.gps = [torch.empty((max_gp,), **f32) for _ in range(2 if side else 1)] if (train and max_gp) else None
        self.gp_turn = 0
        self.gp_free: List[Optional[torch.cuda.Event]] = [None, None]
        self.partials = torch.empty((max_part,), **f32)
        self.conv_ws = torch.empty((max_slab,), **f32) if (train and max_slab) else None
        self.db_sums = torch.empty((65 * 2 * max(u.cin for u in self.units),), device=dev, dtype=torch.float64) if train else None
        self.wgrad_ws = torch.empty((max(max_ws, 64 * max(1, self.n_classes)),), **f32) if train else None
        self.wgrad_ws_side = torch.empty((max(max_ws, 64),), **f32) if side else None
        self.outw_partials = self.outw_sums = None
        if train and self.n_classes > 1:
            kc = self.n_classes * self.dims[0]
            self.outw_partials = torch.empty((lib.gsd_conv1x1_out_wgrad_rows(n, hs[0], ws[0]) * kc,), **f32)
            self.outw_sums = torch.empty((65 * kc,), device=dev, dtype=torch.float64)

    @staticmethod
    def _layouts(jobs, st: int) -> None:
        arr = (L.gsd_wl_job * len(jobs))()
        for i, (mode, w, co, ci, wt) in enumerate(jobs):
            arr[i].w, arr[i].wt, arr[i].mode, arr[i].Co, arr[i].Ci = w.data_ptr(), wt.data_ptr(), mode, co, ci
        check(lib.gsd_weight_layout_batch(arr, len(jobs), st), "weight_layout_batch")

    @staticmethod
    def _act_src(u: _Unit) -> L.gsd_src:
        return L.make_src(u.raw, u.scale, u.shift, relu=True, slack=L.SLACK)

    def _run_unit(self, u: _Unit, srcs: List[L.gsd_src], P: Dict[str, torch.Tensor], train: bool, st: int,
                  keep: bool = False) -> None:
        n = u.raw.shape[0]
        lh, lw = self.hs[u.level], self.ws[u.level]
        u.form_f = u.forms_f[train]
        arr = L.src_array(srcs)
        u.srcs = arr
        dst = L.dst_array([L.make_dst(u.raw)])
        part = self.partials.data_ptr() if train else None
        ev = self._log_begin()
        check(u.form_f.run(self.conv_ws if train else None, arr, len(srcs), u.wt_f.data_ptr(), u.cin, u.cout, dst, 1, part,
                           n, lh, lw, st), "conv3x3")
        self._log_end(ev, u.cout, u.cin, n, lh, lw, u.form_f.algo)
        if train:
            rows = u.form_f.partial_rows(n, lh, lw, u.cout)
            count = float(n * lh * lw)
            if self.sync_fn is None and rows <= self.one_launch_rows:
                check(lib.gsd_bn_reduce_finalize(self.partials.data_ptr(), rows, _r64(u.cout), u.cout, u.sums.data_ptr(), count,
                                                 P[u.gname].data_ptr(), P[u.bname].data_ptr(), BN_EPS, BN_MOMENTUM,
                                                 P[u.rmname].data_ptr(), P[u.rvname].data_ptr(), u.mean.data_ptr(),
                                                 u.invstd.data_ptr(), u.scale.data_ptr(), u.shift.data_ptr(), self.guard, st),
                      "bn_reduce_finalize")
                self._nbt.append(P[u.nbtname])
                return
            check(lib.gsd_bn_reduce_partials(self.partials.data_ptr(), rows, _r64(u.cout), u.cout, u.sums.data_ptr(), st),
                  "bn_reduce_partials")
            if self.sync_fn is not None:
                self.sync_fn(u.sums[:2 * u.cout])
                count *= self.world
            check(lib.gsd_bn_finalize(u.sums.data_ptr(), u.cout, count, P[u.gname].data_ptr(), P[u.bname].data_ptr(),
                                      BN_EPS, BN_MOMENTUM, P[u.rmname].data_ptr(), P[u.rvname].data_ptr(),
                                      u.mean.data_ptr(), u.invstd.data_ptr(), u.scale.data_ptr(), u.shift.data_ptr(),
                                      self.guard, st),
                  "bn_finalize")
            self._nbt.append(P[u.nbtname])
        elif keep:
            check(lib.gsd_bn_eval_coeffs_bwd(P[u.gname].data_ptr(), P[u.bname].data_ptr(), P[u.rmname].data_ptr(),
                                             P[u.rvname].data_ptr(), BN_EPS, u.cout, u.scale.data_ptr(), u.shift.data_ptr(),
                                             u.mean.data_ptr(), u.invstd.data_ptr(), st),
                  "bn_eval_coeffs_bwd")
        else:
            check(lib.gsd_bn_eval_coeffs(P[u.gname].data_ptr(), P[u.bname].data_ptr(), P[u.rmname].data_ptr(),
                                         P[u.rvname].data_ptr(), BN_EPS, u.cout, u.scale.data_ptr(), u.shift.data_ptr(), st),
                  "bn_eval_coeffs")

    def _log_begin(self):
        if self.kernel_log is None and self.region_log is None:
            return None
        e = torch.cuda.Event(enable_timing=True)
        e.record()
        return e

    def _log_end(self, ev, m: int, k_ch: int, n: int, lh: int, lw: int, algo: int = 0) -> None:
        if ev is None or self.kernel_log is None:
            return
        e = torch.cuda.Event(enable_timing=True)
        e.record()
        flops = 2.0 * m * k_ch * 9 * n * lh * lw
        if algo == 2:
            variant = "conv3x3_w2d_kernel"
            executed = 2048.0 * lib.gsd_conv3x3_w2d_mfma_count(n, lh, lw, k_ch, m)
        elif algo:
            variant = "conv3x3_w43_kernel"
            executed = 2048.0 * lib.gsd_conv3x3_w43_mfma_count(n, lh, lw, k_ch, m)
        else:
            variant = "conv3x3_dma_kernel<1,4>" if m <= 64 else "conv3x3_dma_kernel<2,2>"
            executed = flops
        self.kernel_log.append((variant, flops, ev, e, (m, k_ch, lh, lw), executed))

    def _pad_off(self, lvl: int) -> Tuple[int, int]:
        dy = self.hs[lvl] - 2 * self.hs[lvl + 1]
        dx = self.ws[lvl] - 2 * self.ws[lvl + 1]
        return dy // 2, dx // 2

    def forward(self, x: torch.Tensor, P: Dict[str, torch.Tensor], train: bool, out: Optional[torch.Tensor] = None,
                keep: bool = False) -> torch.Tensor:
        if x.dtype != torch.float32 or not x.is_cuda:
            raise L.GsdError("UNetEngine.forward needs a float32 tensor on the GPU (no CPU fallback)")
        self._nbt = []
        x = x.contiguous()
        n, c, h, w = x.shape
        assert c == self.n_channels, f"expected {self.n_channels} input channels, got {c}"
        keep = keep and not train
        self._ensure(n, h, w, x.device, train or keep)
        st = L.stream_ptr()
        self._x = x
        self._saved = train or keep
        self._saved_eval = keep
        self.generation += 1
        self._layouts([(u.forms_f[train].mode_f, P[u.wname], u.cout, u.cin, u.wt_f) for u in self.units] +
                      [(6, P[up.wname], up.cout, up.cin, up.wt_f) for up in self.ups], st)
        region = self._log_begin() if self.region_log is not None else None
        for lvl in range(self.L + 1):
            u0, u1 = self.enc[lvl]
            if lvl == 0:
                srcs = [L.make_src(x)]
            else:
                if lvl == 1 and region is not None:
                    e = torch.cuda.Event(enable_timing=True)
                    e.record()
                    self.region_log.append(("inc_forward", region, e))
                prev = self.enc[lvl - 1][1]
                s = self._act_src(prev)
                check(lib.gsd_maxpool2(C.byref(s), self.pooled[lvl].data_ptr(), n, prev.cout, self.hs[lvl - 1],
                                       self.ws[lvl - 1], st), "maxpool2")
                srcs = [L.make_src(self.pooled[lvl], slack=L.SLACK)]
            self._run_unit(u0, srcs, P, train, st, keep)
            self._run_unit(u1, [self._act_src(u0)], P, train, st, keep)
        if self.L == 0 and region is not None:
            e = torch.cuda.Event(enable_timing=True)
            e.record()
            self.region_log.append(("inc_forward", region, e))
        cur = self.enc[self.L][1]
        for j in range(self.L):
            up = self.ups[j]
            lvl = self.L - 1 - j
            s = self._act_src(cur)
            d = L.make_dst(up.out)
            check(lib.gsd_convT2x2(C.byref(s), up.wt_f.data_ptr(), P[up.bname].data_ptr(), up.cin, up.cout, C.byref(d), n,
                                   self.hs[lvl + 1], self.ws[lvl + 1], st), "convT2x2")
            skip = self.enc[lvl][1]
            u0, u1 = self.dec[j]
            self._run_unit(u0, [self._act_src(skip), L.make_src(up.out, off=self._pad_off(lvl), slack=L.SLACK)], P, train, st,
                           keep)
            self._run_unit(u1, [self._act_src(u0)], P, train, st, keep)
            cur = u1
        if self._nbt:
            L.add_counters(self._nbt, 1)
            self._nbt = []
        if out is None:
            out = torch.empty((n, self.n_classes, h, w), device=x.device, dtype=torch.float32)
        s = self._act_src(cur)
        check(lib.gsd_conv1x1_out(C.byref(s), P["outc.conv.weight"].data_ptr(), P["outc.conv.bias"].data_ptr(), cur.cout,
                                  self.n_classes, out.data_ptr(), n, h, w, st), "conv1x1_out")
        return out

    def _bn_bwd_tail(self, u: _Unit, P, G, st: int, dwout: Optional[torch.Tensor] = None, fused: bool = False) -> None:
        n = u.raw.shape[0]
        lh, lw = self.hs[u.level], self.ws[u.level]
        rows = u.fused_rows if fused else lib.gsd_bn_bwd_partial_rows(n, u.cout, lh, lw)
        count = float(n * lh * lw)
        if self.sync_fn is None and rows <= self.one_launch_rows and (dwout is None or not fused):
            check(lib.gsd_bn_bwd_reduce_finalize(self.partials.data_ptr(), rows, _r64(u.cout) if fused else 0, u.cout,
                                                 u.sums.data_ptr(), count, G[u.gname].data_ptr(), G[u.bname].data_ptr(),
                                                 None if dwout is None else dwout.data_ptr(), u.c1.data_ptr(), u.c2.data_ptr(), st),
                  "bn_bwd_reduce_finalize")
        else:
            if fused:
                check(lib.gsd_bn_reduce_partials(self.partials.data_ptr(), rows, _r64(u.cout), u.cout, u.sums.data_ptr(), st),
                      "bn_reduce_partials")
            else:
                check(lib.gsd_bn_bwd_reduce_partials(self.partials.data_ptr(), rows, u.cout, u.sums.data_ptr(), st),
                      "bn_bwd_reduce_partials")
            gsum = None
            if self.sync_fn is not None:
                gsum = u.sums[:2 * u.cout].clone()
                self.sync_fn(gsum)
                count *= self.world
            check(lib.gsd_bn_bwd_finalize(u.sums.data_ptr(), L.ptr(gsum), u.cout, count, G[u.gname].data_ptr(),
                                          G[u.bname].data_ptr(), None if dwout is None else dwout.data_ptr(),
                                          u.c1.data_ptr(), u.c2.data_ptr(), st),
                  "bn_bwd_finalize")
        if self._saved_eval:
            u.c1.zero_()
            u.c2.zero_()
        if u.fused_dw:
            self._on_side(lambda sst, ws: check(
                lib.gsd_conv3x3_wgrad_bn(u.srcs, u.g.data_ptr(), u.raw.data_ptr(), u.scale.data_ptr(), u.mean.data_ptr(),
                                         u.invstd.data_ptr(), u.c1.data_ptr(), u.c2.data_ptr(), u.cin, u.cout,
                                         G[u.wname].data_ptr(), ws.data_ptr(), ws.numel(), n, lh, lw, sst), "conv3x3_wgrad_bn"))
            return
        turn = None
        if u.pitched:
            p = _r4(lw)
            turn = self.gp_turn = (self.gp_turn + 1) % len(self.gps)
            if self.gp_free[turn] is not None:
                torch.cuda.current_stream().wait_event(self.gp_free[turn])
                self.gp_free[turn] = None
            u.dsrc = self.gps[turn][:n * u.cout * lh * p].view(n, u.cout, lh, p)[..., :lw]
            out_ptr = u.dsrc.data_ptr()
        else:
            p, u.dsrc, out_ptr = 0, u.g, None
        check(lib.gsd_bn_bwd_apply(u.g.data_ptr(), u.raw.data_ptr(), u.scale.data_ptr(), u.mean.data_ptr(),
                                   u.invstd.data_ptr(), u.c1.data_ptr(), u.c2.data_ptr(), n, u.cout, lh, lw, out_ptr, p, st),
              "bn_bwd_apply")
        dy = L.make_src(u.dsrc)
        ev0 = self._log_begin() if self.wgrad_log is not None else None
        on_side = self._on_side(lambda sst, ws: check(
            lib.gsd_conv3x3_wgrad(u.srcs, len(u.srcs), C.byref(dy), u.cin, u.cout, G[u.wname].data_ptr(), ws.data_ptr(), ws.numel(),
                                  n, lh, lw, sst), "conv3x3_wgrad"))
        if ev0 is not None and not on_side:
            ev1 = torch.cuda.Event(enable_timing=True)
            ev1.record()
            form = lib.gsd_conv3x3_wgrad_form(u.srcs, len(u.srcs), C.byref(dy), u.cin, u.cout, n, lh, lw)
            name = ("wgrad3x3_kernel", "wgrad3x3_w43_kernel", "wgrad3x3_w2d_kernel")[form]
            flops = 2.0 * u.cout * u.cin * 9 * n * lh * lw
            executed = 2048.0 * lib.gsd_conv3x3_wgrad_mfma_count(form, n, lh, lw, u.cin, u.cout) if form else flops
            self.wgrad_log.append((name, flops, ev0, ev1, (u.cout, u.cin, lh, lw), executed))
        if on_side and turn is not None:
            self.gp_free[turn] = self.side.record_event()

    def _on_side(self, launch) -> bool:
        if self.side is None or self.kernel_log is not None:
            launch(L.stream_ptr(), self.wgrad_ws)
            return False
        self.side.wait_stream(torch.cuda.current_stream())
        with torch.cuda.stream(self.side):
            launch(L.stream_ptr(), self.wgrad_ws_side)
        return True

    def _join_side(self) -> None:
        if self.side is not None:
            torch.cuda.current_stream().wait_stream(self.side)
            self.gp_free = [None, None]

    def _announce(self, tag: str) -> None:
        if self.block_done_cb is None:
            return
        if self.side is None or self.kernel_log is not None:
            self.block_done_cb(tag)
            return
        if self._handoff is None:
            self._handoff = torch.cuda.Stream(device=self.side.device)
        h = self._handoff
        h.wait_stream(torch.cuda.current_stream())
        h.wait_stream(self.side)
        with torch.cuda.stream(h):
            self.block_done_cb(tag)

    def _reduce(self, mode: int, u: _Unit, st: int, dpool: Optional[torch.Tensor] = None,
                dout: Optional[torch.Tensor] = None, wout: Optional[torch.Tensor] = None) -> None:
        n = u.raw.shape[0]
        lh, lw = self.hs[u.level], self.ws[u.level]
        da = L.make_src(u.g)
        check(lib.gsd_bn_bwd_reduce(mode, u.raw.data_ptr(), u.scale.data_ptr(), u.shift.data_ptr(), u.mean.data_ptr(),
                                    u.invstd.data_ptr(), C.byref(da), L.ptr(dpool), L.ptr(dout), L.ptr(wout),
                                    self.n_classes, u.g.data_ptr(), self.partials.data_ptr(), n, u.cout, lh, lw, st),
              "bn_bwd_reduce")

    def _dgrad(self, u: _Unit, P, dsts: List[L.gsd_dst], st: int, stats: bool = False) -> int:
        n = u.raw.shape[0]
        lh, lw = self.hs[u.level], self.ws[u.level]
        s = L.src_array([L.make_src(u.dsrc)])
        ev = self._log_begin()
        check(u.form_d.run(self.conv_ws, s, 1, u.wt_d.data_ptr(), u.cout, u.cin, L.dst_array(dsts), len(dsts),
                           self.partials.data_ptr() if stats else None, n, lh, lw, st), "conv3x3 dgrad")
        self._log_end(ev, u.cin, u.cout, n, lh, lw, u.form_d.algo)
        return u.form_d.partial_rows(n, lh, lw, u.cin) if stats else 0

    def _dgrad_fused(self, u: _Unit, prev: _Unit, P, st: int) -> None:
        n = u.raw.shape[0]
        lh, lw = self.hs[u.level], self.ws[u.level]
        s = L.make_src(u.dsrc)
        d = L.make_dst(prev.g)
        prev.fused_rows = u.form_d.partial_rows(n, lh, lw, u.cin)
        ev = self._log_begin()
        check(u.form_d.run_bnrelu(self.conv_ws, C.byref(s), u.wt_d.data_ptr(), u.cout, u.cin, C.byref(d), prev.raw.data_ptr(),
                                  prev.scale.data_ptr(), prev.shift.data_ptr(), prev.mean.data_ptr(),
                                  prev.invstd.data_ptr(), self.partials.data_ptr(), n, lh, lw, st),
              "conv3x3_dgrad_bnrelu")
        self._log_end(ev, u.cin, u.cout, n, lh, lw, u.form_d.algo)

    def _input_dgrad(self, u: _Unit, P, dx: torch.Tensor, st: int) -> None:
        n = u.raw.shape[0]
        lh, lw = self.hs[u.level], self.ws[u.level]
        if u.fused_dw:
            check(lib.gsd_conv3x3_dgrad_bn(u.g.data_ptr(), u.raw.data_ptr(), u.scale.data_ptr(), u.mean.data_ptr(),
                                           u.invstd.data_ptr(), u.c1.data_ptr(), u.c2.data_ptr(), P[u.wname].data_ptr(), u.cin,
                                           u.cout, dx.data_ptr(), n, lh, lw, st), "conv3x3_dgrad_bn")
            return
        check(lib.gsd_weight_layout(1, P[u.wname].data_ptr(), u.cout, u.cin, u.wt_d.data_ptr(), st), "weight_layout")
        s = L.src_array([L.make_src(u.dsrc)])
        rc = lib.gsd_conv3x3(s, 1, u.wt_d.data_ptr(), u.cout, u.cin, L.dst_array([L.make_dst(dx)]), 1, None, n, lh, lw, st)
        if rc == GSD_ERR_UNSUPPORTED:
            raise NotImplementedError(f"gelslim_depth_amd.UNet: no kernel computes the input gradient of the first conv3x3 at "
                                      f"N={n} H={lh} W={lw} Cin={u.cin} Cout={u.cout}: "
                                      + lib.gsd_last_error().decode("utf-8", "replace"))
        check(rc, "conv3x3 dgrad (input)")

    def input_grad_supported(self, n: int, h: int, w: int) -> bool:
        u = self.enc[0][0]
        if lib.gsd_conv3x3_wgrad_bn_supported(n, h, w, u.cin, u.cout):
            return bool(lib.gsd_conv3x3_dgrad_bn_supported(n, h, w, u.cin, u.cout))
        return h < 32768 and w < 32768

    def backward(self, dout: torch.Tensor, P: Dict[str, torch.Tensor], G: Dict[str, torch.Tensor],
                 dx: Optional[torch.Tensor] = None) -> None:
        if not self._saved:
            raise L.GsdError("backward() needs a preceding train-mode forward()")
        if self._saved_eval and self.sync_fn is not None:
            raise NotImplementedError("UNetEngine.backward after an eval-mode forward is single-process only (sync_fn is set)")
        if dx is not None:
            x = self._x
            if dx.shape != x.shape or dx.dtype != torch.float32 or not dx.is_contiguous() or dx.device != x.device:
                raise L.GsdError(f"backward(dx=...): expected a contiguous float32 {tuple(x.shape)} tensor on {x.device}")
            u = self.enc[0][0]
            if u.fused_dw and not lib.gsd_conv3x3_dgrad_bn_supported(x.shape[0], x.shape[2], x.shape[3], u.cin, u.cout):
                raise NotImplementedError(f"gelslim_depth_amd.UNet: no kernel computes the input gradient at input shape "
                                          f"{tuple(x.shape)} with {u.cout} first-layer channels")
        dout = dout.contiguous()
        st = L.stream_ptr()
        n = dout.shape[0]
        self._layouts([(u.form_d.mode_d, P[u.wname], u.cout, u.cin, u.wt_d) for u in self.units if u.need_dgrad] +
                      [(up.mode_d, P[up.wname], up.cout, up.cin, up.wt_d) for up in self.ups], st)
        last = self.dec[-1][1] if self.L > 0 else self.enc[0][1]
        self._reduce(2, last, st, dout=dout, wout=P["outc.conv.weight"])
        check(lib.gsd_sum_planes(dout.data_ptr(), n, self.n_classes, dout.shape[2] * dout.shape[3],
                                 G["outc.conv.bias"].data_ptr(), self.wgrad_ws.data_ptr(), st), "sum_planes")
        dwout = G["outc.conv.weight"]
        if self.n_classes > 1:
            lh, lw = self.hs[last.level], self.ws[last.level]
            check(lib.gsd_conv1x1_out_wgrad(last.raw.data_ptr(), last.scale.data_ptr(), last.shift.data_ptr(), dout.data_ptr(),
                                            last.cout, self.n_classes, dwout.data_ptr(), self.outw_partials.data_ptr(),
                                            self.outw_sums.data_ptr(), n, lh, lw, st), "conv1x1_out_wgrad")
            dwout = None
        for j in reversed(range(self.L)):
            u0, u1 = self.dec[j]
            up = self.ups[j]
            lvl = self.L - 1 - j
            self._bn_bwd_tail(u1, P, G, st, dwout, fused=j < self.L - 1 and self.ups[j + 1].bn_rows > 0)
            dwout = None
            self._dgrad_fused(u1, u0, P, st)
            self._bn_bwd_tail(u0, P, G, st, fused=True)
            skip = self.enc[lvl][1]
            db_fused = u0.form_d.algo >= 1
            rows = self._dgrad(u0, P, [L.make_dst(skip.g), L.make_dst(up.dout, off=self._pad_off(lvl))], st, stats=db_fused)
            if db_fused:
                check(lib.gsd_partials_channel_sums(self.partials.data_ptr(), rows, _r64(u0.cin), u0.cin, skip.cout, up.cout,
                                                    G[up.bname].data_ptr(), self.db_sums.data_ptr(), st), "partials_channel_sums")
            prev = self.dec[j - 1][1] if j > 0 else self.enc[self.L][1]
            hi, wi = self.hs[lvl + 1], self.ws[lvl + 1]
            xs = self._act_src(prev)
            dys = L.make_src(up.dout, slack=L.SLACK)
            self._on_side(lambda sst, ws, up=up, xs=xs, dys=dys, db_fused=db_fused, hi=hi, wi=wi: check(
                lib.gsd_convT2x2_wgrad(C.byref(xs), C.byref(dys), up.cin, up.cout, G[up.wname].data_ptr(),
                                       None if db_fused else G[up.bname].data_ptr(), ws.data_ptr(), ws.numel(), n, hi, wi, sst),
                "convT2x2_wgrad"))
            d = L.make_dst(prev.g)
            if up.bn_rows:
                check(lib.gsd_convT2x2_dgrad_bnrelu(C.byref(dys), up.wt_d.data_ptr(), up.cin, up.cout, C.byref(d), prev.raw.data_ptr(),
                                                    prev.scale.data_ptr(), prev.shift.data_ptr(), prev.mean.data_ptr(),
                                                    prev.invstd.data_ptr(), self.partials.data_ptr(), n, hi, wi, st),
                      "convT2x2_dgrad_bnrelu")
                prev.fused_rows = up.bn_rows
            else:
                check(lib.gsd_convT2x2_dgrad_as(up.mode_d, C.byref(dys), up.wt_d.data_ptr(), up.cin, up.cout, C.byref(d), n, hi, wi, st),
                      "convT2x2_dgrad")
                self._reduce(0, prev, st)
            self._announce(f"dec{j}")
        for lvl in reversed(range(self.L + 1)):
            u0, u1 = self.enc[lvl]
            if lvl < self.L:
                self._reduce(1, u1, st, dpool=self.dpooled[lvl + 1])
            self._bn_bwd_tail(u1, P, G, st, dwout, fused=lvl == self.L and self.L > 0 and self.ups[0].bn_rows > 0)
            dwout = None
            self._dgrad_fused(u1, u0, P, st)
            self._bn_bwd_tail(u0, P, G, st, fused=True)
            if lvl == 0 and dx is not None:
                self._input_dgrad(u0, P, dx, st)
            self._announce(f"enc{lvl}")
            if lvl > 0:
                self._dgrad(u0, P, [L.make_dst(self.dpooled[lvl])], st)
        self._join_side()
```

### include/gsd.h

```cpp
#ifndef GSD_H
#define GSD_H

#include <stdint.h>

#ifdef __cplusplus
extern "C" {
#endif

typedef enum {
  GSD_OK = 0,
  GSD_ERR_BAD_ARG = -1,
  GSD_ERR_UNSUPPORTED = -2,
  GSD_ERR_HIP = -3,
  GSD_ERR_WORKSPACE = -4
} gsd_status;

typedef struct {
  int32_t* words;
  int32_t tick;
} gsd_guard;
int gsd_guard_snapshot(const float* live, float* snapshot, int64_t n, void* stream);
int gsd_guard_restore(const gsd_guard* guard, float* live, const float* snapshot, int64_t n, void* stream);

typedef struct {
  const float* ptr;
  const float* scale;
  const float* shift;
  int32_t C;
  int32_t H, W;
  int32_t off_h, off_w;
  int32_t relu;
  int32_t w_stride;
  int32_t slack;
  int64_t n_stride;
  int64_t c_stride;
} gsd_src;

typedef struct {
  float* ptr;
  int32_t C;
  int32_t H, W;
  int32_t off_h, off_w;
  int32_t w_stride;
  int64_t n_stride;
  int64_t c_stride;
} gsd_dst;

const char* gsd_version(void);
const char* gsd_last_error(void);
int gsd_selftest_mfma(const float* a, const float* b, float* out, void* stream);

int64_t gsd_weight_layout_size(int mode, int Co, int Ci);
int gsd_weight_layout(int mode, const float* w, int Co, int Ci, float* wt, void* stream);
typedef struct {
  const float* w;
  float* wt;
  int32_t mode, Co, Ci, reserved;
} gsd_wl_job;
int gsd_weight_layout_batch(const gsd_wl_job* jobs, int n, void* stream);

int gsd_conv3x3_partial_rows(int N, int H, int W, int Cout);
int gsd_conv3x3(const gsd_src* src, int nsrc, const float* wt, int Cin, int Cout,
                const gsd_dst* dst, int ndst, float* partials, int N, int H, int W, void* stream);

int gsd_conv3x3_dgrad_bnrelu(const gsd_src* src, const float* wt, int Cin, int Cout, const gsd_dst* dst,
                             const float* raw, const float* scale, const float* shift, const float* mean,
                             const float* invstd, float* partials, int N, int H, int W, void* stream);

int gsd_conv3x3_algo(int N, int H, int W, int Cin, int Cout);
int gsd_conv3x3_w43_partial_rows(int N, int H, int W, int Cout);
int64_t gsd_conv3x3_w43_mfma_count(int N, int H, int W, int Cin, int Cout);
int gsd_conv3x3_w43(const gsd_src* src, int nsrc, const float* wt, int Cin, int Cout,
                    const gsd_dst* dst, int ndst, float* partials, int N, int H, int W, void* stream);
int gsd_conv3x3_w43_dgrad_bnrelu(const gsd_src* src, const float* wt, int Cin, int Cout, const gsd_dst* dst,
                                 const float* raw, const float* scale, const float* shift, const float* mean,
                                 const float* invstd, float* partials, int N, int H, int W, void* stream);
int64_t gsd_conv3x3_w43_workspace(int N, int H, int W, int Cin, int Cout);
int gsd_conv3x3_w43_ws(const gsd_src* src, int nsrc, const float* wt, int Cin, int Cout, const gsd_dst* dst, int ndst,
                       float* partials, float* ws, int64_t ws_elems, int N, int H, int W, void* stream);
int gsd_conv3x3_w43_dgrad_bnrelu_ws(const gsd_src* src, const float* wt, int Cin, int Cout, const gsd_dst* dst,
                                    const float* raw, const float* scale, const float* shift, const float* mean,
                                    const float* invstd, float* partials, float* ws, int64_t ws_elems, int N, int H, int W,
                                    void* stream);

int gsd_conv3x3_w2d_supported(int Cin, int C0);
int gsd_conv3x3_prefers_w2d(int N, int H, int W, int Cin, int Cout, int train);
double gsd_conv3x3_w2d_estimate_us(int N, int H, int W, int Cin, int Cout);
double gsd_conv3x3_w43_estimate_us(int N, int H, int W, int Cin, int Cout, int slabs);
int gsd_conv3x3_w2d_partial_rows(int N, int H, int W, int Cout);
int64_t gsd_conv3x3_w2d_mfma_count(int N, int H, int W, int Cin, int Cout);
int gsd_conv3x3_w2d(const gsd_src* src, int nsrc, const float* wt, int Cin, int Cout,
                    const gsd_dst* dst, int ndst, float* partials, int N, int H, int W, void* stream);
int gsd_conv3x3_w2d_dgrad_bnrelu(const gsd_src* src, const float* wt, int Cin, int Cout, const gsd_dst* dst,
                                 const float* raw, const float* scale, const float* shift, const float* mean,
                                 const float* invstd, float* partials, int N, int H, int W, void* stream);
double gsd_conv3x3_w2d_estimate_slabs_us(int N, int H, int W, int Cin, int Cout);
int64_t gsd_conv3x3_w2d_workspace(int N, int H, int W, int Cin, int Cout);
int gsd_conv3x3_w2d_ws(const gsd_src* src, int nsrc, const float* wt, int Cin, int Cout, const gsd_dst* dst, int ndst,
                       float* partials, float* workspace, int64_t workspace_elems, int N, int H, int W, void* stream);
int gsd_conv3x3_w2d_dgrad_bnrelu_ws(const gsd_src* src, const float* wt, int Cin, int Cout, const gsd_dst* dst,
                                    const float* raw, const float* scale, const float* shift, const float* mean,
                                    const float* invstd, float* partials, float* workspace, int64_t workspace_elems,
                                    int N, int H, int W, void* stream);

int gsd_convT2x2(const gsd_src* src, const float* wt, const float* bias, int Cin, int Cout,
                 const gsd_dst* dst, int N, int H, int W, void* stream);
int gsd_convT2x2_dgrad_layout(const gsd_src* src, int Cin, int Cout, int N, int H, int W);
int gsd_convT2x2_dgrad(const gsd_src* src, const float* wt, int Cin, int Cout,
                       const gsd_dst* dst, int N, int H, int W, void* stream);
int gsd_convT2x2_dgrad_as(int wt_mode, const gsd_src* src, const float* wt, int Cin, int Cout,
                          const gsd_dst* dst, int N, int H, int W, void* stream);
int gsd_convT2x2_dgrad_bnrelu_partial_rows(const gsd_src* src, int Cin, int Cout, int N, int H, int W);
int gsd_convT2x2_dgrad_bnrelu(const gsd_src* src, const float* wt, int Cin, int Cout, const gsd_dst* dst, const float* raw,
                              const float* scale, const float* shift, const float* mean, const float* invstd,
                              float* partials, int N, int H, int W, void* stream);

int64_t gsd_conv3x3_wgrad_workspace(int N, int H, int W, int Cin, int Cout);
int gsd_conv3x3_wgrad(const gsd_src* a, int nsrc, const gsd_src* dy, int Cin, int Cout,
                      float* dw, float* workspace, int64_t workspace_elems,
                      int N, int H, int W, void* stream);
int gsd_conv3x3_wgrad_form(const gsd_src* a, int nsrc, const gsd_src* dy, int Cin, int Cout, int N, int H, int W);
int64_t gsd_conv3x3_wgrad_mfma_count(int form, int N, int H, int W, int Cin, int Cout);
int gsd_conv3x3_wgrad_takes_pitched_dy(int N, int H, int W, int Cin, int Cout);
int gsd_conv3x3_wgrad_bn_supported(int N, int H, int W, int Cin, int Cout);
int64_t gsd_conv3x3_wgrad_bn_workspace(int N, int H, int W, int Cin, int Cout);
int gsd_conv3x3_wgrad_bn(const gsd_src* a, const float* dz, const float* raw, const float* scale,
                         const float* mean, const float* invstd, const float* c1, const float* c2,
                         int Cin, int Cout, float* dw, float* workspace, int64_t workspace_elems,
                         int N, int H, int W, void* stream);
int gsd_conv3x3_dgrad_bn_supported(int N, int H, int W, int Cin, int Cout);
int gsd_conv3x3_dgrad_bn(const float* dz, const float* raw, const float* scale, const float* mean,
                         const float* invstd, const float* c1, const float* c2, const float* w,
                         int Cin, int Cout, float* dx, int N, int H, int W, void* stream);
int64_t gsd_convT2x2_wgrad_workspace(int N, int H, int W, int Cin, int Cout);
int gsd_convT2x2_wgrad(const gsd_src* x, const gsd_src* dy, int Cin, int Cout,
                       float* dw, float* dbias, float* workspace, int64_t workspace_elems,
                       int N, int H, int W, void* stream);

int gsd_bn_reduce_partials(const float* partials, int rows, int Mpad, int C, double* sums, void* stream);
int gsd_partials_channel_sums(const float* partials, int rows, int Mpad, int C, int c_begin, int c_count, float* out,
                              double* sums, void* stream);
int gsd_add_counters(int64_t* const* counters, int n, int64_t delta, void* stream);
int gsd_bn_finalize(const double* sums, int C, double count, const float* gamma, const float* beta,
                    float eps, float momentum, float* running_mean, float* running_var,
                    float* mean, float* invstd, float* scale, float* shift, const gsd_guard* guard, void* stream);
int gsd_bn_eval_coeffs(const float* gamma, const float* beta, const float* running_mean,
                       const float* running_var, float eps, int C, float* scale, float* shift, void* stream);

int gsd_bn_eval_coeffs_bwd(const float* gamma, const float* beta, const float* running_mean,
                           const float* running_var, float eps, int C, float* scale, float* shift,
                           float* mean, float* invstd, void* stream);

int gsd_bn_bwd_partial_rows(int N, int C, int H, int W);
int gsd_bn_bwd_reduce(int mode, const float* raw, const float* scale, const float* shift,
                      const float* mean, const float* invstd,
                      const gsd_src* da, const float* dpool, const float* dout, const float* wout,
                      int K, float* dz, float* partials, int N, int C, int H, int W, void* stream);
int gsd_bn_bwd_reduce_partials(const float* partials, int rows, int C, double* sums, void* stream);
int gsd_bn_bwd_finalize(const double* sums_local, const double* sums_global, int C, double count,
                        float* dgamma, float* dbeta, float* dwout, float* c1, float* c2, void* stream);

int gsd_bn_reduce_finalize(const float* partials, int rows, int Mpad, int C, double* sums, double count, const float* gamma,
                           const float* beta, float eps, float momentum, float* running_mean, float* running_var,
                           float* mean, float* invstd, float* scale, float* shift, const gsd_guard* guard, void* stream);
int gsd_bn_bwd_reduce_finalize(const float* partials, int rows, int layout_mpad, int C, double* sums, double count,
                               float* dgamma, float* dbeta, float* dwout, float* c1, float* c2, void* stream);
int gsd_bn_bwd_apply(float* dz, const float* raw, const float* scale, const float* mean,
                     const float* invstd, const float* c1, const float* c2,
                     int N, int C, int H, int W, float* out, int out_w_stride, void* stream);
int gsd_sum_planes(const float* x, int N, int K, int64_t HW, float* out, float* workspace, void* stream);

int gsd_maxpool2(const gsd_src* src, float* y, int N, int C, int H, int W, void* stream);

int gsd_conv1x1_out(const gsd_src* src, const float* w, const float* b, int C, int K,
                    float* out, int N, int H, int W, void* stream);
int gsd_conv1x1_out_wgrad_rows(int N, int H, int W);
int gsd_conv1x1_out_wgrad(const float* raw, const float* scale, const float* shift, const float* dout, int C, int K,
                          float* dw, float* partials, double* sums, int N, int H, int W, void* stream);
int gsd_loss_fwd_bwd(int kind, const float* o, const float* t, int64_t numel, float grad_scale,
                     float* loss_out, float* grad, float* workspace, const gsd_guard* guard, void* stream);

int gsd_adam_ema(float* p, const float* g, float* m, float* v, float* ema, int64_t numel,
                 int step, float lr, float beta1, float beta2, float eps, float weight_decay,
                 float ema_decay, float grad_scale, const gsd_guard* guard, void* stream);

int gsd_area_resize_affine(const float* in, const float* base, int N, int C, int H, int W, float* out, int OH, int OW,
                           const float* A, const float* B, int nab, float pre_add, float pre_mul, void* stream);

typedef enum {
  GSD_INTERP_AREA = 0,
  GSD_INTERP_NEAREST = 1,
  GSD_INTERP_NEAREST_EXACT = 2,
  GSD_INTERP_BILINEAR = 3,
  GSD_INTERP_BICUBIC = 4
} gsd_interp;
int gsd_resize_affine(int mode, const float* in, const float* base, int N, int C, int H, int W, float* out, int OH, int OW,
                      const float* A, const float* B, int nab, float pre_add, float pre_mul, void* stream);

int gsd_ingest_images(const void* in, const void* base, int dtype, int N, int C, int H, int W, int64_t in_n_stride,
                      int64_t in_c_stride, int64_t base_n_stride, int64_t base_c_stride, float* out, int OH, int OW,
                      float pre_add, float pre_mul, void* stream);
int gsd_ingest_images_interp(int mode, const void* in, const void* base, int dtype, int N, int C, int H, int W,
                             int64_t in_n_stride, int64_t in_c_stride, int64_t base_n_stride, int64_t base_c_stride, float* out,
                             int OH, int OW, float pre_add, float pre_mul, void* stream);
int gsd_gaussian_blur(const float* in, int64_t planes, int H, int W, const float* kernel2d, int K, float* out, void* stream);
int64_t gsd_channel_stats_workspace(int C);
int gsd_channel_stats(const float* x, int64_t N, int C, int64_t HW, double* out, double* workspace, void* stream);
int gsd_gather_affine(const float* src, const int64_t* idx, int64_t M, int B, int C, int64_t HW, const float* A,
                      const float* Bc, int nab, float* out, void* stream);

#ifdef __cplusplus
}
#endif
#endif
```

Before: 369.8.

## Fold batch images into tile rows for w2d conv in training

Adds a folded tiling mode to the w2d 3x3 conv kernel in which row tiles run across image boundaries, treating the N images as one tall image with a seam. This cuts the partially filled edge tiles that per-image tiling leaves when H does not divide evenly into the tile height. The fold is chosen only in training, and only when a cost model predicts fewer blocks and a lower time. It adds an extra window row, index logic at the seam and a separate kernel instantiation, with a 31-bit stride limit check.

```diff
diff --git a/gelslim_depth_amd/_lib.py b/gelslim_depth_amd/_lib.py
--- a/gelslim_depth_amd/_lib.py
+++ b/gelslim_depth_amd/_lib.py
@@ -90,6 +90,12 @@
     "gsd_conv3x3_w2d_workspace": (_L, [_I, _I, _I, _I, _I]),
     "gsd_conv3x3_w2d_ws": (_I, [_SRC, _I, _P, _I, _I, _DST, _I, _P, _P, _L, _I, _I, _I, _P]),
     "gsd_conv3x3_w2d_dgrad_bnrelu_ws": (_I, [_SRC, _P, _I, _I, _DST, _P, _P, _P, _P, _P, _P, _P, _L, _I, _I, _I, _P]),
+    "gsd_conv3x3_w2d_train": (_I, [_SRC, _I, _P, _I, _I, _DST, _I, _P, _P, _L, _I, _I, _I, _P]),
+    "gsd_conv3x3_w2d_dgrad_bnrelu_train": (_I, [_SRC, _P, _I, _I, _DST, _P, _P, _P, _P, _P, _P, _P, _L, _I, _I, _I, _P]),
+    "gsd_conv3x3_w2d_train_folds": (_I, [_I, _I, _I, _I, _I]),
+    "gsd_conv3x3_w2d_train_partial_rows": (_I, [_I, _I, _I, _I, _I]),
+    "gsd_conv3x3_w2d_train_mfma_count": (C.c_int64, [_I, _I, _I, _I, _I]),
+    "gsd_conv3x3_w2d_train_workspace": (_L, [_I, _I, _I, _I, _I]),
     "gsd_conv3x3_w43_workspace": (_L, [_I, _I, _I, _I, _I]),
     "gsd_conv3x3_w43_ws": (_I, [_SRC, _I, _P, _I, _I, _DST, _I, _P, _P, _L, _I, _I, _I, _P]),
     "gsd_conv3x3_w43_dgrad_bnrelu_ws": (_I, [_SRC, _P, _I, _I, _DST, _P, _P, _P, _P, _P, _P, _P, _L, _I, _I, _I, _P]),
diff --git a/gelslim_depth_amd/csrc/gsd_conv3x3_w2d.hip b/gelslim_depth_amd/csrc/gsd_conv3x3_w2d.hip
--- a/gelslim_depth_amd/csrc/gsd_conv3x3_w2d.hip
+++ b/gelslim_depth_amd/csrc/gsd_conv3x3_w2d.hip
@@ -22,6 +22,7 @@
   int Cin, Cout, Mpad, nchunks, mblocks;
   int N, H, W;
   int TH, TW, TWq, tiles_y, tiles_x, WR, WC, WCp, PS, NPV;
+  int fold;
   int NP, NI;
   int mgrp, pgrp, ptiles;
   int nslab;
@@ -35,9 +36,9 @@
 }
 
 template <class GetY>
-__device__ __forceinline__ void w2d_epilogue(const W2DParams& P, const float* sBw, const int n, const int h0, const int w0, const int tr2,
-                                             const int tq, const int vmask, const int m0, const int mh, const int ph, const int j,
-                                             const int l16, const int pt, GetY get_y) {
+__device__ __forceinline__ void w2d_epilogue(const W2DParams& P, const float* sBw, const int n, const int dn, const int h0, const int w0,
+                                             const int tr2, const int tq, const int vmask, const int m0, const int mh, const int ph,
+                                             const int j, const int l16, const int pt, GetY get_y) {
   constexpr int BM = 64;
   int off0_0 = 0, off0_1 = 0, off1_0 = 0, off1_1 = 0, sm0_0 = 0, sm0_1 = 0, sm1_0 = 0, sm1_1 = 0;
 #pragma unroll
@@ -64,7 +65,7 @@
   auto OFF1 = [&](int a) { return a == 0 ? off1_0 : off1_1; };
   auto SM0 = [&](int a) { return a == 0 ? sm0_0 : sm0_1; };
   auto SM1 = [&](int a) { return a == 0 ? sm1_0 : sm1_1; };
-  const long long lane0 = (long long)(j * 4) * P.dst0.cs, lane1 = (long long)(j * 4) * P.dst1.cs;
+  const long long lane0 = (long long)(j * 4) * P.dst0.cs + (dn ? P.dst0.ns : 0), lane1 = (long long)(j * 4) * P.dst1.cs + (dn ? P.dst1.ns : 0);
   float* const d0 = P.dst0.p + (long long)n * P.dst0.ns;
   float* const d1 = P.dst1.p + (long long)n * P.dst1.ns;
   float* const prow = P.partials != nullptr ? P.partials + (size_t)(pt * NWP + ph) * (2 * P.Mpad) : nullptr;
@@ -117,7 +118,7 @@
 #pragma unroll
       for (int reg = 0; reg < 4; ++reg) {
         const int cu = m0 + mh * 32 + m * 16 + reg, co = cu + j * 4;
-        const long long cplane = (long long)n * P.dst0.ns + (co < P.Cout ? (long long)cu * P.dst0.cs + lane0 : 0);
+        const long long cplane = (long long)n * P.dst0.ns + (co < P.Cout ? (long long)cu * P.dst0.cs + lane0 : (dn ? P.dst0.ns : 0));
         float xr[2][4];
 #pragma unroll
         for (int a = 0; a < 2; ++a) {
@@ -168,8 +169,8 @@
   }
 }
 
-template <bool PLAIN, int HM = 0, bool SPLIT = false>
-__global__ __launch_bounds__(128 * NWP, 2) void conv3x3_w2d_kernel(const W2DParams P) {
+template <bool PLAIN, int HM, bool SPLIT, bool FOLD>
+__device__ __forceinline__ void w2d_block(const W2DParams P) {
   constexpr bool X4 = HM == 1, U4 = HM == 2, PC = HM != 0;
   constexpr int W2D_NONE = -2147483647 - 1, W2D_PAD = -2147483647;
   static_assert(!X4 || PLAIN, "aligned 16-byte halo pieces: a plain, row-pitched source");
@@ -205,29 +206,45 @@
   const int c_hi = SPLIT ? (int)((long)(slab + 1) * P.nchunks / P.nslab) : P.nchunks;
   const int m0 = mbb * BM;
   const int tpi = P.tiles_y * P.tiles_x;
-  const int n = pt / tpi;
-  const int rt = pt - n * tpi;
+  const int n_pt = pt / tpi;
+  const int rt = pt - n_pt * tpi;
   const int ty = rt / P.tiles_x;
-  const int h0 = ty * P.TH, w0 = (rt - ty * P.tiles_x) * P.TW;
+  const int w0 = (rt - ty * P.tiles_x) * P.TW;
+  const int nf = FOLD ? ty * P.TH / P.H : 0;
+  const int n = FOLD ? nf : n_pt, h0 = ty * P.TH - nf * P.H;
 
   const int q = ph * 16 + l16;
   const bool q_ok = q < (P.TH >> 1) * P.TWq && q < 16 * NWP;
   const int tr2 = q_ok ? q / P.TWq : 0;
   const int tq = q_ok ? q - tr2 * P.TWq : 0;
-  const int baddr = WTILE + j * PS + (2 * tr2) * P.WCp + 4 * tq + (PC ? 4 : 0);
+  const int dn0 = FOLD && h0 + 2 * tr2 >= P.H ? 1 : 0;
+  const int baddr = WTILE + j * PS + (2 * tr2 + dn0) * P.WCp + 4 * tq + (PC ? 4 : 0);
   int vmask = 0;
   if (q_ok) {
 #pragma unroll
     for (int a = 0; a < 2; ++a)
-      if (h0 + 2 * tr2 + a < P.H) {
+      if (h0 - dn0 * P.H + 2 * tr2 + a < P.H && (!FOLD || n + dn0 < P.N)) {
 #pragma unroll
         for (int i = 0; i < 4; ++i)
           if (w0 + 4 * tq + i < P.W) vmask |= 1 << (4 * a + i);
       }
   }
+  if constexpr (FOLD) vmask |= dn0 << 8;
 
   bool p_on[2];
   int pmask = 0;
+  auto win_row = [&](const int rr, const SrcD& S, int& io) __attribute__((always_inline)) {
+    int gh = h0 - 1 + rr;
+    io = 0;
+    if constexpr (FOLD) {
+      if (gh > P.H) {
+        gh -= P.H + 1;
+        io = (int)S.ns;
+        if (n + 1 >= P.N) gh = -65536;
+      }
+    }
+    return gh;
+  };
   auto seg_offsets = [&](const int seg, int (&xo)[2], const bool mark) __attribute__((always_inline)) {
     const SrcD& S = seg ? P.src1 : P.src0;
 #pragma unroll
@@ -239,14 +256,15 @@
         const int piece = (u % P.NI) * 64 + lane;
         const int rr = piece / P.NP, pc = piece - rr * P.NP;
         if (rr < P.WR) {
-          const int gh = h0 - 1 + rr, gw = w0 - 4 + 4 * pc;
+          int io;
+          const int gh = win_row(rr, S, io), gw = w0 - 4 + 4 * pc;
           if constexpr (X4) {
-            xo[pp] = ((unsigned)gh < (unsigned)S.H && gw >= 0 && gw + 4 <= S.ws) ? gh * S.ws + gw : W2D_PAD;
+            xo[pp] = ((unsigned)gh < (unsigned)S.H && gw >= 0 && gw + 4 <= S.ws) ? io + gh * S.ws + gw : W2D_PAD;
           } else {
             const int hs = gh - S.oh, c0 = gw - S.ow;
             xo[pp] = W2D_PAD;
             if (S.C > 0 && (unsigned)hs < (unsigned)S.H && c0 + 3 >= 0 && c0 < S.W) {
-              xo[pp] = hs * S.ws + c0;
+              xo[pp] = io + hs * S.ws + c0;
 #pragma unroll
               for (int e = 0; e < 4; ++e)
                 if (mark && (c0 + e < 0 || c0 + e >= S.W)) pmask |= 1 << (8 * seg + 4 * pp + e);
@@ -259,9 +277,10 @@
       const int pos = (wave8 + NW * pp) * 64 + lane;
       const int rr = pos / P.WCp, cc = pos - rr * P.WCp;
       if (rr < P.WR && cc < P.WC) {
-        const int gh = h0 - 1 + rr, gw = w0 - 1 + cc;
+        int io;
+        const int gh = win_row(rr, S, io), gw = w0 - 1 + cc;
         const int hs = gh - S.oh, ws = gw - S.ow;
-        xo[pp] = ((unsigned)hs < (unsigned)S.H && (unsigned)ws < (unsigned)S.W) ? hs * S.ws + ws : W2D_PAD;
+        xo[pp] = ((unsigned)hs < (unsigned)S.H && (unsigned)ws < (unsigned)S.W) ? io + hs * S.ws + ws : W2D_PAD;
       }
     }
   };
@@ -573,13 +592,32 @@
           *reinterpret_cast<f32x4*>(o + 4) = f32x4{y[1][0], y[1][1], y[1][2], y[1][3]};
         }
     } else {
-      w2d_epilogue(P, sBw, n, h0, w0, tr2, tq, vmask, m0, fh, ph, j, l16, pt, get_y);
+      if constexpr (FOLD) {
+        int vm = vmask, te = tid;
+        __asm__ volatile("" : "+v"(vm), "+v"(te));
+        const int dn = vm >> 8, le = te & 63, qe = ph * 16 + (le & 15);
+        const bool qe_ok = qe < (P.TH >> 1) * P.TWq && qe < 16 * NWP;
+        const int tr2e = qe_ok ? qe / P.TWq : 0, tqe = qe_ok ? qe - tr2e * P.TWq : 0;
+        w2d_epilogue(P, sBw, n, dn, h0 - dn * P.H, w0, tr2e, tqe, vm & 255, m0, fh, ph, le >> 4, le & 15, pt, get_y);
+      } else {
+        w2d_epilogue(P, sBw, n, 0, h0, w0, tr2, tq, vmask, m0, fh, ph, j, l16, pt, get_y);
+      }
     }
   };
   if (fh == 0)
     finish(std::false_type{});
   else
     finish(std::true_type{});
+}
+
+template <bool PLAIN, int HM = 0, bool SPLIT = false>
+__global__ __launch_bounds__(128 * NWP, 2) void conv3x3_w2d_kernel(const W2DParams P) {
+  w2d_block<PLAIN, HM, SPLIT, false>(P);
+}
+
+template <bool PLAIN, int HM = 0, bool SPLIT = false>
+__global__ __launch_bounds__(128 * NWP, 2) void conv3x3_w2d_fold_kernel(const W2DParams P) {
+  w2d_block<PLAIN, HM, SPLIT, true>(P);
 }
 
 __global__ __launch_bounds__(128 * NWP) void w2d_slab_reduce_kernel(const W2DParams P) {
@@ -594,19 +632,23 @@
   const int pt = lid / P.mblocks;
   const int m0 = mbb * BM;
   const int tpi = P.tiles_y * P.tiles_x;
-  const int n = pt / tpi;
-  const int rt = pt - n * tpi;
+  const int n_pt = pt / tpi;
+  const int rt = pt - n_pt * tpi;
   const int ty = rt / P.tiles_x;
-  const int h0 = ty * P.TH, w0 = (rt - ty * P.tiles_x) * P.TW;
+  const int w0 = (rt - ty * P.tiles_x) * P.TW;
+  const int nf = P.fold ? ty * P.TH / P.H : 0;
+  const int n = P.fold ? nf : n_pt, h0 = ty * P.TH - nf * P.H;
   const int q = ph * 16 + l16;
   const bool q_ok = q < (P.TH >> 1) * P.TWq && q < 16 * NWP;
   const int tr2 = q_ok ? q / P.TWq : 0;
   const int tq = q_ok ? q - tr2 * P.TWq : 0;
+  const int dn = P.fold && h0 + 2 * tr2 >= P.H ? 1 : 0;
+  const int h0l = dn ? h0 - P.H : h0;
   int vmask = 0;
   if (q_ok) {
 #pragma unroll
     for (int a = 0; a < 2; ++a)
-      if (h0 + 2 * tr2 + a < P.H) {
+      if (h0l + 2 * tr2 + a < P.H && n + dn < P.N) {
 #pragma unroll
         for (int i = 0; i < 4; ++i)
           if (w0 + 4 * tq + i < P.W) vmask |= 1 << (4 * a + i);
@@ -635,13 +677,16 @@
     y[0][0] = a[0], y[0][1] = a[1], y[0][2] = a[2], y[0][3] = a[3];
     y[1][0] = b[0], y[1][1] = b[1], y[1][2] = b[2], y[1][3] = b[3];
   };
-  w2d_epilogue(P, sBw, n, h0, w0, tr2, tq, vmask, m0, mh, ph, j, l16, pt, get_y);
+  w2d_epilogue(P, sBw, n, dn, h0l, w0, tr2, tq, vmask, m0, mh, ph, j, l16, pt, get_y);
 }
 
 namespace {
 
 struct W2DPlan {
   int TH, TW, TWq, tiles_y, tiles_x, mblocks, WR, WC, WCp, PS;
+  int fold;
+  long ptiles;
+  long utiles;
 };
 
 int w2d_read_cycles(int TWq, int LP, int PS) {
@@ -688,8 +733,9 @@
   return total;
 }
 
-bool plan_w2d(int N, int H, int W, int M, W2DPlan* best) {
+bool plan_w2d(int N, int H, int W, int M, W2DPlan* best, bool fold = false) {
   long best_cost = -1;
+  if (fold && (N < 2 || H % 2 != 0)) return false;
   const int force_tw = gsd_env_int("GSD_W2D_TW", 0);
   const int maxpos = 256 * NWP;
   static const int tws[4] = {32, 64, 16, 8};
@@ -699,23 +745,26 @@
     const int twq = tw / 4;
     int th = 2 * (16 * NWP / twq);
     const int wcp0 = round_up(tw + 2, 4);
-    if ((th + 2) * wcp0 > maxpos) continue;
-    const int ty = ceil_div(H, th);
-    th = round_up(ceil_div(H, ty), 2);
-    const long blocks = (long)ty * ceil_div(W, tw) * N;
+    if ((th + (fold ? 3 : 2)) * wcp0 > maxpos) continue;
+    if (fold && th > H) continue;
+    const int ty = fold ? ceil_div(N * H, th) : ceil_div(H, th);
+    if (!fold) th = round_up(ceil_div(H, ty), 2);
+    const long blocks = fold ? (long)ty * ceil_div(W, tw) : (long)ty * ceil_div(W, tw) * N;
     const long cost = (blocks * 8 + (tw == 32 ? 0 : tw == 64 ? 1 : tw == 16 ? 2 : 3)) * (tw == 8 ? 100 + gsd_env_int("GSD_W2D_TW8_PCT", 8) : 100);
     if (best_cost < 0 || cost < best_cost) {
       best_cost = cost;
       best->TH = th; best->TW = tw; best->TWq = twq;
       best->tiles_y = ty; best->tiles_x = ceil_div(W, tw);
-      best->WR = th + 2; best->WC = tw + 2;
+      best->WR = th + (fold ? 3 : 2); best->WC = tw + 2;
+      best->fold = fold ? 1 : 0;
+      best->ptiles = best->utiles = blocks;
     }
   }
   best->mblocks = ceil_div(M, W2D_BM);
   if (best_cost < 0) return false;
   static std::atomic<uint64_t> memo[16];
-  const int th = best->TH, tw = best->TW, key = (th << 16) | (tw << 4);
-  std::atomic<uint64_t>& mm = memo[(th * 7 + tw) & 15];
+  const int th = best->TH, tw = best->TW, wr = best->WR, key = (th << 16) | (tw << 4) | best->fold;
+  std::atomic<uint64_t>& mm = memo[(th * 7 + tw + best->fold) & 15];
   {
     const uint64_t v = mm.load(std::memory_order_acquire);
     if (v != 0 && (int)(v >> 40) == key) {
@@ -726,8 +775,8 @@
   }
   const int wcp0 = round_up(tw + 2, 4);
   int bc = -1;
-  for (int c = wcp0; c <= wcp0 + 12 && (th + 2) * c <= maxpos; c += 4)
-    for (int ps = round_up((th + 2) * c, 4) + 4; ps < round_up((th + 2) * c, 4) + 4 + 36; ps += 4) {
+  for (int c = wcp0; c <= wcp0 + 12 && wr * c <= maxpos; c += 4)
+    for (int ps = round_up(wr * c, 4) + 4; ps < round_up(wr * c, 4) + 4 + 36; ps += 4) {
       const int cyc = w2d_read_cycles(best->TWq, c, ps);
       if (bc < 0 || cyc < bc) {
         bc = cyc;
@@ -762,14 +811,14 @@
 
 template <bool PLAIN, int HM = 0, bool SPLIT = false>
 int launch_w2d(const W2DParams& P, int grid, size_t lds, hipStream_t st) {
-  static gsd_attr_once big_lds;
-  const void* fn = reinterpret_cast<const void*>(&conv3x3_w2d_kernel<PLAIN, HM, SPLIT>);
-  if (hipError_t e = gsd_allow_big_lds(big_lds, fn); e != hipSuccess) {
+  static gsd_attr_once big_lds[2];
+  void (*const kern)(const W2DParams) = P.fold ? &conv3x3_w2d_fold_kernel<PLAIN, HM, SPLIT> : &conv3x3_w2d_kernel<PLAIN, HM, SPLIT>;
+  if (hipError_t e = gsd_allow_big_lds(big_lds[P.fold ? 1 : 0], reinterpret_cast<const void*>(kern)); e != hipSuccess) {
     gsd_set_error("gsd_conv3x3_w2d: hipFuncSetAttribute: %s", hipGetErrorString(e));
     return GSD_ERR_HIP;
   }
   GSD_REQUIRE(lds <= 160 * 1024, GSD_ERR_UNSUPPORTED, "gsd_conv3x3_w2d: LDS image %zu B too large", lds);
-  hipLaunchKernelGGL((conv3x3_w2d_kernel<PLAIN, HM, SPLIT>), dim3(grid), dim3(128 * NWP), lds, st, P);
+  hipLaunchKernelGGL(kern, dim3(grid), dim3(128 * NWP), lds, st, P);
   GSD_LAUNCH_CHECK("gsd_conv3x3_w2d");
   if constexpr (SPLIT) {
     hipLaunchKernelGGL(w2d_slab_reduce_kernel, dim3(grid / P.nslab), dim3(128 * NWP), 0, st, P);
@@ -803,6 +852,22 @@
   return best;
 }
 
+bool plan_w2d_train(int N, int H, int W, int Cin, int Cout, W2DPlan* pl) {
+  if (!plan_w2d(N, H, W, Cout, pl)) return false;
+  const int sw = gsd_env_int("GSD_W2D_FOLD", -1);
+  W2DPlan pf;
+  if (sw == 0 || !plan_w2d(N, H, W, Cout, &pf, true)) return true;
+  const long bu = pl->ptiles * pl->mblocks, bf = pf.ptiles * pf.mblocks;
+  if (bf >= bu) return true;
+  if (sw != 1) {
+    const int nch = ceil_div(Cin, 4), S = w2d_pick_slabs(bu, nch, false);
+    if (!(w2d_time_us(bf, nch, S, false) < w2d_time_us(bu, nch, S, false))) return true;
+  }
+  pf.utiles = pl->ptiles;
+  *pl = pf;
+  return true;
+}
+
 }
 
 extern "C" int gsd_conv3x3_w2d_supported(int Cin, int C0) {
@@ -857,7 +922,7 @@
 
 static int w2d_impl(const gsd_src* src, int nsrc, const float* wt, int Cin, int Cout, const gsd_dst* dst, int ndst, float* partials,
                     const float* bw_raw, const float* bw_scale, const float* bw_shift, const float* bw_mean, const float* bw_invstd,
-                    int N, int H, int W, void* stream, float* ws = nullptr, int64_t ws_elems = 0) {
+                    int N, int H, int W, void* stream, float* ws = nullptr, int64_t ws_elems = 0, bool train = false) {
   GSD_REQUIRE(src && dst && wt, GSD_ERR_BAD_ARG, "gsd_conv3x3_w2d: null argument");
   GSD_REQUIRE(nsrc >= 1 && nsrc <= 2 && ndst >= 1 && ndst <= 2, GSD_ERR_BAD_ARG, "gsd_conv3x3_w2d: nsrc/ndst must be 1 or 2");
   GSD_REQUIRE(N > 0 && H > 0 && W > 0 && Cin > 0 && Cout > 0, GSD_ERR_BAD_ARG, "gsd_conv3x3_w2d: bad sizes");
@@ -883,7 +948,12 @@
   GSD_REQUIRE(csum == Cout, GSD_ERR_BAD_ARG, "gsd_conv3x3_w2d: destination segments hold %d channels, Cout=%d", csum, Cout);
 
   W2DPlan pl;
-  GSD_REQUIRE(plan_w2d(N, H, W, Cout, &pl), GSD_ERR_UNSUPPORTED, "gsd_conv3x3_w2d: no tile shape");
+  GSD_REQUIRE(train ? plan_w2d_train(N, H, W, Cin, Cout, &pl) : plan_w2d(N, H, W, Cout, &pl), GSD_ERR_UNSUPPORTED,
+              "gsd_conv3x3_w2d: no tile shape");
+  if (pl.fold)
+    for (int i = 0; i < nsrc; ++i)
+      GSD_REQUIRE(src[i].n_stride + (int64_t)src[i].H * src[i].w_stride < (1LL << 31), GSD_ERR_UNSUPPORTED,
+                  "gsd_conv3x3_w2d: image stride too large for folded tile rows (GSD_W2D_FOLD=0)");
   W2DParams P;
   P.src0 = to_srcd(src[0]);
   P.src1 = nsrc > 1 ? to_srcd(src[1]) : null_srcd();
@@ -899,6 +969,7 @@
   P.N = N; P.H = H; P.W = W;
   P.TH = pl.TH; P.TW = pl.TW; P.TWq = pl.TWq; P.tiles_y = pl.tiles_y; P.tiles_x = pl.tiles_x;
   P.WR = pl.WR; P.WC = pl.WC; P.WCp = pl.WCp; P.PS = pl.PS;
+  P.fold = pl.fold;
   P.NPV = ceil_div(P.WR * P.WCp, 64);
   GSD_REQUIRE(P.NPV <= 4 * NWP, GSD_ERR_UNSUPPORTED, "gsd_conv3x3_w2d: halo window too large");
   {
@@ -908,11 +979,11 @@
     if (forced > 0) g = forced;
     P.mgrp = std::min(std::max(g, 1), P.mblocks);
     P.pgrp = std::max(gsd_env_int("GSD_W2D_PGROUP", 64 / P.mgrp), 1);
-    P.ptiles = N * pl.tiles_y * pl.tiles_x;
-  }
-  const long base = (long)N * pl.tiles_y * pl.tiles_x * P.mblocks;
-  int S = ws != nullptr ? w2d_pick_slabs(base, P.nchunks, bw_raw != nullptr) : 1;
-  while (S > 1 && (int64_t)base * S * (W2D_BM * 256) > ws_elems) --S;
+    P.ptiles = (int)pl.ptiles;
+  }
+  const long base = pl.ptiles * P.mblocks, ubase = pl.utiles * P.mblocks;
+  int S = ws != nullptr ? w2d_pick_slabs(ubase, P.nchunks, bw_raw != nullptr) : 1;
+  while (S > 1 && (int64_t)ubase * S * (W2D_BM * 256) > ws_elems) --S;
   if (S > 1 && P.nchunks / S < 2) S = 1;
   P.nslab = S;
   P.slabs = S > 1 ? ws : nullptr;
@@ -934,9 +1005,9 @@
   }
   const size_t lds = (size_t)(2 * (W2D_WTILE + 4 * P.PS) + 2 * 4 * P.nchunks + 4 * W2D_BM) * sizeof(float);
   if (gsd_env_set("GSD_W2D_TRACE"))
-    fprintf(stderr, "w2d M%d K%d %dx%d N%d nsrc %d ndst %d plain %d x4 %d u4 %d | ptr&15 %d ws %d cs%%4 %d ns%%4 %d NI %d tile %dx%d slabs %d\n", Cout, Cin, H, W, N,
+    fprintf(stderr, "w2d M%d K%d %dx%d N%d nsrc %d ndst %d plain %d x4 %d u4 %d | ptr&15 %d ws %d cs%%4 %d ns%%4 %d NI %d tile %dx%d slabs %d fold %d blocks %ld\n", Cout, Cin, H, W, N,
             nsrc, ndst, (int)plain, (int)x4, (int)u4, (int)((uintptr_t)src[0].ptr & 15), src[0].w_stride, (int)(src[0].c_stride % 4),
-            (int)(src[0].n_stride % 4), P.NI, pl.TH, pl.TW, S);
+            (int)(src[0].n_stride % 4), P.NI, pl.TH, pl.TW, S, pl.fold, base);
   if (S > 1) {
     if (x4) return launch_w2d<true, 1, true>(P, (int)grid, lds, (hipStream_t)stream);
     if (u4) return plain ? launch_w2d<true, 2, true>(P, (int)grid, lds, (hipStream_t)stream) : launch_w2d<false, 2, true>(P, (int)grid, lds, (hipStream_t)stream);
@@ -978,3 +1049,47 @@
               "gsd_conv3x3_w2d_dgrad_bnrelu: dst must be the full (Cout,H,W) gradient buffer (raw shares its strides)");
   return w2d_impl(src, 1, wt, Cin, Cout, dst, 1, partials, raw, scale, shift, mean, invstd, N, H, W, stream, workspace, workspace_elems);
 }
+
+extern "C" int gsd_conv3x3_w2d_train(const gsd_src* src, int nsrc, const float* wt, int Cin, int Cout, const gsd_dst* dst, int ndst,
+                                     float* partials, float* workspace, int64_t workspace_elems, int N, int H, int W, void* stream) {
+  return w2d_impl(src, nsrc, wt, Cin, Cout, dst, ndst, partials, nullptr, nullptr, nullptr, nullptr, nullptr, N, H, W, stream, workspace,
+                  workspace_elems, true);
+}
+
+extern "C" int gsd_conv3x3_w2d_dgrad_bnrelu_train(const gsd_src* src, const float* wt, int Cin, int Cout, const gsd_dst* dst,
+                                                  const float* raw, const float* scale, const float* shift, const float* mean,
+                                                  const float* invstd, float* partials, float* workspace, int64_t workspace_elems,
+                                                  int N, int H, int W, void* stream) {
+  GSD_REQUIRE(dst && raw && scale && shift && mean && invstd && partials, GSD_ERR_BAD_ARG,
+              "gsd_conv3x3_w2d_dgrad_bnrelu: null argument");
+  GSD_REQUIRE(dst->C == Cout && dst->H == H && dst->W == W && dst->off_h == 0 && dst->off_w == 0, GSD_ERR_BAD_ARG,
+              "gsd_conv3x3_w2d_dgrad_bnrelu: dst must be the full (Cout,H,W) gradient buffer (raw shares its strides)");
+  return w2d_impl(src, 1, wt, Cin, Cout, dst, 1, partials, raw, scale, shift, mean, invstd, N, H, W, stream, workspace, workspace_elems,
+                  true);
+}
+
+extern "C" int gsd_conv3x3_w2d_train_folds(int N, int H, int W, int Cin, int Cout) {
+  W2DPlan p;
+  if (N <= 0 || H <= 0 || W <= 0 || Cin <= 0 || Cout <= 0 || !plan_w2d_train(N, H, W, Cin, Cout, &p)) return 0;
+  return p.fold;
+}
+
+extern "C" int gsd_conv3x3_w2d_train_partial_rows(int N, int H, int W, int Cin, int Cout) {
+  W2DPlan p;
+  if (N <= 0 || H <= 0 || W <= 0 || Cin <= 0 || Cout <= 0 || !plan_w2d_train(N, H, W, Cin, Cout, &p)) return 0;
+  return (int)p.ptiles * NWP;
+}
+
+extern "C" int64_t gsd_conv3x3_w2d_train_mfma_count(int N, int H, int W, int Cin, int Cout) {
+  W2DPlan p;
+  if (N <= 0 || H <= 0 || W <= 0 || Cin <= 0 || Cout <= 0 || !plan_w2d_train(N, H, W, Cin, Cout, &p)) return 0;
+  return (int64_t)p.ptiles * p.mblocks * ceil_div(Cin, 4) * (2 * NWP * 48);
+}
+
+extern "C" int64_t gsd_conv3x3_w2d_train_workspace(int N, int H, int W, int Cin, int Cout) {
+  W2DPlan p;
+  if (N <= 0 || H <= 0 || W <= 0 || Cin <= 0 || Cout <= 0 || Cin % 4 != 0 || !plan_w2d_train(N, H, W, Cin, Cout, &p)) return 0;
+  const long blocks = p.utiles * p.mblocks;
+  const int S = std::max(w2d_pick_slabs(blocks, Cin / 4, false), w2d_pick_slabs(blocks, Cin / 4, true));
+  return S > 1 ? (int64_t)blocks * S * (W2D_BM * 256) : 0;
+}
diff --git a/gelslim_depth_amd/engine.py b/gelslim_depth_amd/engine.py
--- a/gelslim_depth_amd/engine.py
+++ b/gelslim_depth_amd/engine.py
@@ -55,6 +55,25 @@
             fn = lib.gsd_conv3x3_w43_dgrad_bnrelu_ws if self.algo == 1 else lib.gsd_conv3x3_w2d_dgrad_bnrelu_ws
             return fn(src, wt, cin, cout, dst, raw, scale, shift, mean, invstd, part, ws.data_ptr(), ws.numel(), n, h, w, st)
         return self.dgrad_bnrelu(src, wt, cin, cout, dst, raw, scale, shift, mean, invstd, part, n, h, w, st)
+
+    def train_rows(self, n, h, w, cin, cout):
+        return lib.gsd_conv3x3_w2d_train_partial_rows(n, h, w, cin, cout) if self.algo == 2 else self.partial_rows(n, h, w, cout)
+
+    def train_workspace(self, n, h, w, cin, cout):
+        return lib.gsd_conv3x3_w2d_train_workspace(n, h, w, cin, cout) if self.algo == 2 else self.workspace(n, h, w, cin, cout)
+
+    def run_train(self, ws, src, nsrc, wt, cin, cout, dst, ndst, part, n, h, w, st):
+        if self.algo != 2:
+            return self.run(ws, src, nsrc, wt, cin, cout, dst, ndst, part, n, h, w, st)
+        return lib.gsd_conv3x3_w2d_train(src, nsrc, wt, cin, cout, dst, ndst, part, None if ws is None else ws.data_ptr(),
+                                         0 if ws is None else ws.numel(), n, h, w, st)
+
+    def run_bnrelu_train(self, ws, src, wt, cin, cout, dst, raw, scale, shift, mean, invstd, part, n, h, w, st):
+        if self.algo != 2:
+            return self.run_bnrelu(ws, src, wt, cin, cout, dst, raw, scale, shift, mean, invstd, part, n, h, w, st)
+        return lib.gsd_conv3x3_w2d_dgrad_bnrelu_train(src, wt, cin, cout, dst, raw, scale, shift, mean, invstd, part,
+                                                      None if ws is None else ws.data_ptr(), 0 if ws is None else ws.numel(),
+                                                      n, h, w, st)
 
 
 class _Unit:
@@ -133,7 +152,7 @@
         self.wgrad_log: Optional[list] = None
         self.region_log: Optional[list] = None
 
-    _SIZING_ENV = ("GSD_W2D_TW", "GSD_W2D_TW8_PCT", "GSD_W43_TW", "GSD_W43_FOLD", "GSD_CONV_W2D", "GSD_CONV_ALGO", "GSD_W43_SPLIT",
+    _SIZING_ENV = ("GSD_W2D_TW", "GSD_W2D_TW8_PCT", "GSD_W2D_FOLD", "GSD_W43_TW", "GSD_W43_FOLD", "GSD_CONV_W2D", "GSD_CONV_ALGO", "GSD_W43_SPLIT",
                    "GSD_WGRAD_ALGO", "GSD_WGRAD_W2D", "GSD_WG2D_KX", "GSD_WG2D_BLOCKS", "GSD_WGRAD_BLOCKS", "GSD_WG43_TW")
 
     def _ensure(self, n: int, h: int, w: int, dev: torch.device, train: bool) -> None:
@@ -182,12 +201,15 @@
                 need = lib.gsd_weight_layout_size(u.form_d.mode_d, u.cout, u.cin)
                 if u.wt_d is None or u.wt_d.numel() != need or u.wt_d.device != dev:
                     u.wt_d = torch.empty((need,), **f32)
-                max_part = max(max_part, u.form_d.partial_rows(n, lh, lw, u.cin) * 2 * _r64(u.cin))
-            rows = max(f.partial_rows(n, lh, lw, u.cout) for f in u.forms_f.values())
+                max_part = max(max_part, max(u.form_d.partial_rows(n, lh, lw, u.cin),
+                                             u.form_d.train_rows(n, lh, lw, u.cout, u.cin)) * 2 * _r64(u.cin))
+            rows = max(max(f.partial_rows(n, lh, lw, u.cout), f.train_rows(n, lh, lw, u.cin, u.cout)) for f in u.forms_f.values())
             max_part = max(max_part, rows * 2 * _r64(u.cout))
             if train:
-                max_slab = max(max_slab, u.form_f.workspace(n, lh, lw, u.cin, u.cout),
-                               u.form_d.workspace(n, lh, lw, u.cout, u.cin) if u.need_dgrad else 0)
+                max_slab = max(max_slab, u.form_f.workspace(n, lh, lw, u.cin, u.cout), u.form_f.train_workspace(n, lh, lw, u.cin, u.cout))
+                if u.need_dgrad:
+                    max_slab = max(max_slab, u.form_d.workspace(n, lh, lw, u.cout, u.cin),
+                                   u.form_d.train_workspace(n, lh, lw, u.cout, u.cin))
                 max_part = max(max_part, lib.gsd_bn_bwd_partial_rows(n, u.cout, lh, lw) * 3 * u.cout)
                 max_ws = max(max_ws, lib.gsd_conv3x3_wgrad_workspace(n, lh, lw, u.cin, u.cout))
                 u.pitched = bool(lib.gsd_conv3x3_wgrad_takes_pitched_dy(n, lh, lw, u.cin, u.cout)) and \
@@ -257,11 +279,12 @@
         dst = L.dst_array([L.make_dst(u.raw)])
         part = self.partials.data_ptr() if train else None
         ev = self._log_begin()
-        check(u.form_f.run(self.conv_ws if train else None, arr, len(srcs), u.wt_f.data_ptr(), u.cin, u.cout, dst, 1, part,
-                           n, lh, lw, st), "conv3x3")
-        self._log_end(ev, u.cout, u.cin, n, lh, lw, u.form_f.algo)
+        run = u.form_f.run_train if train else u.form_f.run
+        check(run(self.conv_ws if train else None, arr, len(srcs), u.wt_f.data_ptr(), u.cin, u.cout, dst, 1, part,
+                  n, lh, lw, st), "conv3x3")
+        self._log_end(ev, u.cout, u.cin, n, lh, lw, u.form_f.algo, train)
         if train:
-            rows = u.form_f.partial_rows(n, lh, lw, u.cout)
+            rows = u.form_f.train_rows(n, lh, lw, u.cin, u.cout)
             count = float(n * lh * lw)
             if self.sync_fn is None and rows <= self.one_launch_rows:
                 check(lib.gsd_bn_reduce_finalize(self.partials.data_ptr(), rows, _r64(u.cout), u.cout, u.sums.data_ptr(), count,
@@ -299,7 +322,7 @@
         e.record()
         return e
 
-    def _log_end(self, ev, m: int, k_ch: int, n: int, lh: int, lw: int, algo: int = 0) -> None:
+    def _log_end(self, ev, m: int, k_ch: int, n: int, lh: int, lw: int, algo: int = 0, train: bool = False) -> None:
         if ev is None or self.kernel_log is None:
             return
         e = torch.cuda.Event(enable_timing=True)
@@ -307,7 +330,8 @@
         flops = 2.0 * m * k_ch * 9 * n * lh * lw
         if algo == 2:
             variant = "conv3x3_w2d_kernel"
-            executed = 2048.0 * lib.gsd_conv3x3_w2d_mfma_count(n, lh, lw, k_ch, m)
+            count = lib.gsd_conv3x3_w2d_train_mfma_count if train else lib.gsd_conv3x3_w2d_mfma_count
+            executed = 2048.0 * count(n, lh, lw, k_ch, m)
         elif algo:
             variant = "conv3x3_w43_kernel"
             executed = 2048.0 * lib.gsd_conv3x3_w43_mfma_count(n, lh, lw, k_ch, m)
@@ -491,23 +515,29 @@
         lh, lw = self.hs[u.level], self.ws[u.level]
         s = L.src_array([L.make_src(u.dsrc)])
         ev = self._log_begin()
-        check(u.form_d.run(self.conv_ws, s, 1, u.wt_d.data_ptr(), u.cout, u.cin, L.dst_array(dsts), len(dsts),
-                           self.partials.data_ptr() if stats else None, n, lh, lw, st), "conv3x3 dgrad")
-        self._log_end(ev, u.cin, u.cout, n, lh, lw, u.form_d.algo)
-        return u.form_d.partial_rows(n, lh, lw, u.cin) if stats else 0
+        train = not self._saved_eval
+        run = u.form_d.run_train if train else u.form_d.run
+        check(run(self.conv_ws, s, 1, u.wt_d.data_ptr(), u.cout, u.cin, L.dst_array(dsts), len(dsts),
+                  self.partials.data_ptr() if stats else None, n, lh, lw, st), "conv3x3 dgrad")
+        self._log_end(ev, u.cin, u.cout, n, lh, lw, u.form_d.algo, train)
+        if not stats:
+            return 0
+        return u.form_d.train_rows(n, lh, lw, u.cout, u.cin) if train else u.form_d.partial_rows(n, lh, lw, u.cin)
 
     def _dgrad_fused(self, u: _Unit, prev: _Unit, P, st: int) -> None:
         n = u.raw.shape[0]
         lh, lw = self.hs[u.level], self.ws[u.level]
         s = L.make_src(u.dsrc)
         d = L.make_dst(prev.g)
-        prev.fused_rows = u.form_d.partial_rows(n, lh, lw, u.cin)
+        train = not self._saved_eval
+        prev.fused_rows = u.form_d.train_rows(n, lh, lw, u.cout, u.cin) if train else u.form_d.partial_rows(n, lh, lw, u.cin)
         ev = self._log_begin()
-        check(u.form_d.run_bnrelu(self.conv_ws, C.byref(s), u.wt_d.data_ptr(), u.cout, u.cin, C.byref(d), prev.raw.data_ptr(),
+        run = u.form_d.run_bnrelu_train if train else u.form_d.run_bnrelu
+        check(run(self.conv_ws, C.byref(s), u.wt_d.data_ptr(), u.cout, u.cin, C.byref(d), prev.raw.data_ptr(),
                                   prev.scale.data_ptr(), prev.shift.data_ptr(), prev.mean.data_ptr(),
                                   prev.invstd.data_ptr(), self.partials.data_ptr(), n, lh, lw, st),
               "conv3x3_dgrad_bnrelu")
-        self._log_end(ev, u.cin, u.cout, n, lh, lw, u.form_d.algo)
+        self._log_end(ev, u.cin, u.cout, n, lh, lw, u.form_d.algo, train)
 
     def _input_dgrad(self, u: _Unit, P, dx: torch.Tensor, st: int) -> None:
         n = u.raw.shape[0]
diff --git a/include/gsd.h b/include/gsd.h
--- a/include/gsd.h
+++ b/include/gsd.h
@@ -102,6 +102,16 @@
                                     const float* raw, const float* scale, const float* shift, const float* mean,
                                     const float* invstd, float* partials, float* workspace, int64_t workspace_elems,
                                     int N, int H, int W, void* stream);
+int gsd_conv3x3_w2d_train(const gsd_src* src, int nsrc, const float* wt, int Cin, int Cout, const gsd_dst* dst, int ndst,
+                          float* partials, float* workspace, int64_t workspace_elems, int N, int H, int W, void* stream);
+int gsd_conv3x3_w2d_dgrad_bnrelu_train(const gsd_src* src, const float* wt, int Cin, int Cout, const gsd_dst* dst,
+                                       const float* raw, const float* scale, const float* shift, const float* mean,
+                                       const float* invstd, float* partials, float* workspace, int64_t workspace_elems,
+                                       int N, int H, int W, void* stream);
+int gsd_conv3x3_w2d_train_folds(int N, int H, int W, int Cin, int Cout);
+int gsd_conv3x3_w2d_train_partial_rows(int N, int H, int W, int Cin, int Cout);
+int64_t gsd_conv3x3_w2d_train_mfma_count(int N, int H, int W, int Cin, int Cout);
+int64_t gsd_conv3x3_w2d_train_workspace(int N, int H, int W, int Cin, int Cout);
 
 int gsd_convT2x2(const gsd_src* src, const float* wt, const float* bias, int Cin, int Cout,
                  const gsd_dst* dst, int N, int H, int W, void* stream);
```

Result: faster. 375.1 (median of 6 runs) (+1.4%).
